# kamerkaya/SUPerman

Measured on AMD Instinct MI355X. Metric: Gray-code subset-steps/sec (dense n=40, d=0.5) at 1/2/4/8 MI355X; rel-err vs CPU, higher is better.
Workload: dtype f64; 1 GPU; dense Ryser/Gray-code exact permanent (-p4/-p6 path), n=40 d=0.50 (double/40_0.50_0), 2^39 Gray steps per step; n=40, kernel_request=dense, preprocessing=0, jit=1, walk=segmented (pattern-specialised), parallelism=dp1: contiguous wave-chunk shards + one RCCL all-reduce

## Files before the change

### include/superman.h

```cpp
#ifndef SUPERMAN_H
#define SUPERMAN_H

#include <stddef.h>
#include <stdint.h>

#ifdef __cplusplus
extern "C" {
#endif

#define SUP_ABI_VERSION 15

#define SUP_OK            0
#define SUP_EINVAL      (-1)
#define SUP_ENODEV      (-2)
#define SUP_EHIP        (-3)
#define SUP_ERCCL       (-4)
#define SUP_ENOMEM      (-5)
#define SUP_EIO         (-6)
#define SUP_EUNSUPPORTED (-7)

#define SUP_MAX_N 64
#define SUP_MAX_READ_N 4096

typedef enum {
  SUP_INT32 = 0,
  SUP_FLOAT32 = 1,
  SUP_FLOAT64 = 2
} sup_dtype;

typedef enum {
  SUP_KERNEL_DENSE = 0,
  SUP_KERNEL_SPARYSER = 1,
  SUP_KERNEL_SKIPPER = 2,
  SUP_KERNEL_DENSE_PLAIN = 3,
  SUP_KERNEL_SEGMENTED = 4,
  SUP_KERNEL_DENSE_LDS = 5
} sup_kernel;

typedef enum {
  SUP_SCHED_SINGLE = 0,
  SUP_SCHED_STATIC = 1,
  SUP_SCHED_CHUNKS = 2,
  SUP_SCHED_MANUAL = 3
} sup_sched;

typedef struct {
  int gpu_num;
  int device_id;
  int threads;
  int cpu_worker;
  int grid_dim;
  int block_dim;
  int walk_log2;
  int chunk_log2;
  int use_rccl;
  int verbose;
  int jit;
  const char* checkpoint;
  int timing;
} sup_opts;

typedef struct {
  double   kernel_ms;
  double   wall_ms;
  uint64_t gray_steps;
  uint64_t visited_steps;
  int      devices_used;
  int      lane_bits;
  int      walk_bits;
  int      grid;
  int      chunks_done_cpu;
  double   partials[16];
  int      walk_kind;
  int      leaves;
  double   est_ops_per_step;
  double   jit_ms;
  int      items_resumed;
  int16_t  seg_cached_bits;
  int16_t  seg_pair_bits;
} sup_stats;

void sup_opts_init(sup_opts* o);

int         sup_abi_version(void);
const char* sup_last_error(void);
int         sup_device_count(int* count);
int         sup_rccl_devices(int ndev, int* phys);
uint64_t    sup_device_checks(void);
int         sup_device_warmup(int device_id, int gpu_num, int n);
int         sup_kernel_time(int device_id, double* total_ms, uint64_t* launches);

int sup_perman(const void* mat, sup_dtype t, int n, sup_kernel kernel, sup_sched sched,
               const sup_opts* o, double* out, sup_stats* st);

int sup_partial(const void* mat, sup_dtype t, int n, sup_kernel kernel,
                uint64_t start, uint64_t end, const sup_opts* o, double* out, sup_stats* st);

int sup_perman_shard(const void* mat, sup_dtype t, int n, sup_kernel kernel, int shard, int nshards,
                     const sup_opts* o, double* out_partial, sup_stats* st);

int sup_plan_info(const void* mat, sup_dtype t, int n, sup_kernel kernel, const sup_opts* o, int* walk_kind,
                  int* colmap, int* lane_bits, int* walk_bits, int* cached_bits, int* pair_bits,
                  double* est_ops_per_step);

int sup_plan_key(const void* mat, sup_dtype t, int n, sup_kernel kernel, const sup_opts* o, uint64_t* key);

int sup_prepare(const void* mat, sup_dtype t, int n, sup_kernel kernel, const sup_opts* o, int* walk_kind,
                double* compile_ms);
int sup_perman_cpu(const void* mat, sup_dtype t, int n, sup_kernel kernel, int threads,
                   double* out, sup_stats* st);

int sup_perman_exact(const void* mat, sup_dtype t, int n, const sup_opts* o, int on_cpu, char* out,
                     size_t out_len, sup_stats* st);

int sup_perman_exact_range(const void* mat, sup_dtype t, int n, uint64_t c0, uint64_t c1, const sup_opts* o,
                           int on_cpu, int form, int group, uint64_t* primes, uint64_t* residues, int cap,
                           int* nprimes, int* colmap, sup_stats* st);

int sup_perman_quad(const void* mat, sup_dtype t, int n, const sup_opts* o, int on_cpu, double* out_hi,
                    double* out_lo, sup_stats* st);

int sup_perman_quad_range(const void* mat, sup_dtype t, int n, uint64_t c0, uint64_t c1, const sup_opts* o,
                          int on_cpu, int form, double* out_hi, double* out_lo, int* colmap, sup_stats* st);

int sup_perman_complex(const double* mat, int n, const sup_opts* o, int on_cpu,
                       double* out_re, double* out_im, sup_stats* st);
int sup_perman_complex_range(const double* mat, int n, uint64_t c0, uint64_t c1,
                             const sup_opts* o, int on_cpu,
                             double* out_re, double* out_im, sup_stats* st);

int sup_perman_complex_batch(const double* mats, int n, uint64_t count, const sup_opts* o,
                             int on_cpu, double* out, sup_stats* st);
int sup_perman_complex_submatrices(const double* U, int R, int C, const int32_t* rows,
                                   const int32_t* cols, int n, uint64_t count, const sup_opts* o,
                                   int on_cpu, double* out, sup_stats* st);

int sup_perman_complex_fock(const double* U, int R, int C, const int32_t* rows,
                            const int32_t* cols, int n, uint64_t count, const sup_opts* o,
                            int on_cpu, double* out, sup_stats* st);
int sup_perman_complex_fock_plan(const int32_t* rows, const int32_t* cols, int n,
                                 uint64_t count, uint64_t* terms, int* side);

int sup_perman_complex_minors(const double* U, int R, int C, const int32_t* rows, const int32_t* cols,
                              int n, uint64_t count, const sup_opts* o, int on_cpu, double* out, sup_stats* st);
int sup_perman_complex_minors_range(const double* mat, int n, uint64_t c0, uint64_t c1, const sup_opts* o,
                                    int on_cpu, double* out, sup_stats* st);
int sup_boson_sample(const double* U, int M, const int32_t* inputs, int n, uint64_t nsamples, uint64_t seed,
                     const sup_opts* o, int on_cpu, int32_t* out , sup_stats* st);

int sup_nw_start(const void* mat, sup_dtype t, int n, double* x0, double* p0);


int sup_gpu_perman64_xshared_coalescing_mshared(const void* mat, sup_dtype t, int nov,
    int grid_dim, int block_dim, double* out);
int sup_gpu_perman64_xshared_coalescing_mshared_multigpu(const void* mat, sup_dtype t, int nov,
    int gpu_num, int grid_dim, int block_dim, double* out);
int sup_gpu_perman64_xshared_coalescing_mshared_multigpucpu_chunks(const void* mat, sup_dtype t,
    int nov, int gpu_num, int cpu, int threads, int grid_dim, int block_dim, double* out);
int sup_gpu_perman64_xshared_coalescing_mshared_sparse(const void* mat, const int* cptrs,
    const int* rows, const void* cvals, sup_dtype t, int nov, int grid_dim, int block_dim,
    double* out);
int sup_gpu_perman64_xshared_coalescing_mshared_multigpu_sparse(const void* mat, const int* cptrs,
    const int* rows, const void* cvals, sup_dtype t, int nov, int gpu_num, int grid_dim,
    int block_dim, double* out);
int sup_gpu_perman64_xshared_coalescing_mshared_multigpucpu_chunks_sparse(const void* mat,
    const int* cptrs, const int* rows, const void* cvals, sup_dtype t, int nov, int gpu_num,
    int cpu, int threads, int grid_dim, int block_dim, double* out);
int sup_gpu_perman64_xshared_coalescing_mshared_multigpu_manual_distribution(const void* mat, sup_dtype t,
    int nov, int gpu_num, int grid_dim, int block_dim, double* out);
int sup_gpu_perman64_xshared_coalescing_mshared_multigpu_sparse_manual_distribution(const void* mat,
    const int* cptrs, const int* rows, const void* cvals, sup_dtype t, int nov, int gpu_num, int grid_dim,
    int block_dim, double* out);
int sup_gpu_perman64_xshared_coalescing_mshared_skipper(const void* mat, const int* rptrs,
    const int* cols, const int* cptrs, const int* rows, const void* cvals, sup_dtype t, int nov,
    int grid_dim, int block_dim, double* out);
int sup_gpu_perman64_xshared_coalescing_mshared_multigpucpu_chunks_skipper(const void* mat,
    const int* rptrs, const int* cols, const int* cptrs, const int* rows, const void* cvals,
    sup_dtype t, int nov, int gpu_num, int cpu, int threads, int grid_dim, int block_dim,
    double* out);


int sup_read_matrix(const char* path, int binary, void** mat, sup_dtype* t, int* n, int* nnz_header);
void sup_free(void* p);

int sup_count_nnz(const void* mat, sup_dtype t, int n, int* nnz);
int sup_compress(const void* mat, sup_dtype t, int n, int* cptrs, int* rows, void* cvals,
                 int* rptrs, int* cols, void* rvals);
int sup_sort_order(void* mat, sup_dtype t, int n, int* colperm);
int sup_skip_order(void* mat, sup_dtype t, int n, int* rowperm, int* colperm);

int sup_read_mtx(const char* path, int binary, void** mat, sup_dtype* t, int* n, int* nnz_lines);
int sup_read_mtx_complex(const char* path, double** mat, int* n, int* nnz_lines);

typedef struct {
  int compress;
  double scale_threshold;
  int min_n;
  int max_deg;
  int preprocessing;
} sup_reduce_opts;
void sup_reduce_opts_init(sup_reduce_opts* r);

typedef int (*sup_leaf_fn)(const double* a, int n, void* user, double* out_perm);

int sup_decompose(const void* mat, sup_dtype t, int n, const sup_reduce_opts* r, sup_leaf_fn fn, void* user,
                  double* out, int* n_leaves);

int sup_perman_reduced(const void* mat, sup_dtype t, int n, sup_kernel kernel, sup_sched sched, const sup_opts* o,
                       int on_cpu, const sup_reduce_opts* r, double* out, sup_stats* st);

int sup_perman_reduced_exact(const void* mat, sup_dtype t, int n, const sup_opts* o, int on_cpu,
                             const sup_reduce_opts* r, char* out, size_t out_len, sup_stats* st);

int sup_perman_reduced_quad(const void* mat, sup_dtype t, int n, const sup_opts* o, int on_cpu,
                            const sup_reduce_opts* r, double* out_hi, double* out_lo, sup_stats* st);



typedef struct {
  double   mean;
  double   std_error;
  double   zero_fraction;
  uint64_t samples;
  double   kernel_ms;
  double   wall_ms;
  int      devices;
  int      reserved_;
  int64_t  cpu_blocks;
} sup_approx_result;

int sup_approx(const void* mat, sup_dtype t, int n, int method, uint64_t samples, int scale_intervals,
               int scale_times, uint64_t seed, const sup_opts* o, int on_cpu, sup_approx_result* res);

int sup_grid_graph(int m, int n, int** mat, int* nov);

#ifdef __cplusplus
}
#endif
#endif
```

### superman_amd/__init__.py

```python
from __future__ import annotations

import ctypes as C
import os

import numpy as np

from . import _lib
from ._lib import (KERNEL_DENSE, KERNEL_SKIPPER, KERNEL_SPARYSER, LEAF_FN, SCHED_CHUNKS, SCHED_MANUAL, SCHED_SINGLE,
                   SCHED_STATIC, SupApproxResult, SupError, SupOpts, SupReduceOpts, SupStats)

__all__ = [
    "perman", "perman_cpu", "perman_exact", "perman_exact_range", "perman_quad", "perman_quad_range", "perman_complex", "perman_complex_range", "perman_complex_batch", "perman_complex_submatrices", "perman_complex_fock", "perman_complex_fock_plan", "perman_complex_minors", "perman_complex_minors_submatrices", "perman_complex_minors_range", "boson_sample", "read_mtx_complex", "partial", "perman_shard", "plan_info", "plan_key", "prepare", "read_matrix", "read_mtx", "sort_order",
    "skip_order", "compress", "decompose", "perman_reduced", "approx", "grid_graph", "ALGOS_APPROX",
    "nw_start", "device_count", "rccl_devices", "layout", "ShardCall", "SupError", "ALGOS_DENSE", "ALGOS_SPARSE",
    "gpu_perman64_xshared_coalescing_mshared",
    "gpu_perman64_xshared_coalescing_mshared_multigpu",
    "gpu_perman64_xshared_coalescing_mshared_multigpucpu_chunks",
    "gpu_perman64_xshared_coalescing_mshared_sparse",
    "gpu_perman64_xshared_coalescing_mshared_multigpu_sparse",
    "gpu_perman64_xshared_coalescing_mshared_multigpucpu_chunks_sparse",
    "gpu_perman64_xshared_coalescing_mshared_skipper",
    "gpu_perman64_xshared_coalescing_mshared_multigpucpu_chunks_skipper",
]

_DT = {np.dtype(np.int32): _lib.SUP_INT32, np.dtype(np.float32): _lib.SUP_FLOAT32,
       np.dtype(np.float64): _lib.SUP_FLOAT64}
_NP = {_lib.SUP_INT32: np.int32, _lib.SUP_FLOAT32: np.float32, _lib.SUP_FLOAT64: np.float64}
_TYPE_NAME = {_lib.SUP_INT32: "int", _lib.SUP_FLOAT32: "float", _lib.SUP_FLOAT64: "double"}

ALGOS_DENSE = {
    0: ("gpu_perman64_xglobal", KERNEL_DENSE, SCHED_SINGLE),
    1: ("gpu_perman64_xlocal", KERNEL_DENSE, SCHED_SINGLE),
    2: ("gpu_perman64_xshared", KERNEL_DENSE, SCHED_SINGLE),
    3: ("gpu_perman64_xshared_coalescing", KERNEL_DENSE, SCHED_SINGLE),
    4: ("gpu_perman64_xshared_coalescing_mshared", KERNEL_DENSE, SCHED_SINGLE),
    5: ("gpu_perman64_xshared_coalescing_mshared_multigpu", KERNEL_DENSE, SCHED_STATIC),
    6: ("gpu_perman64_xshared_coalescing_mshared_multigpucpu_chunks", KERNEL_DENSE, SCHED_CHUNKS),
    66: ("gpu_perman64_xshared_coalescing_mshared_multigpu_manual_distribution", KERNEL_DENSE, SCHED_MANUAL),
}
ALGOS_SPARSE = {
    1: ("gpu_perman64_xlocal_sparse", KERNEL_SPARYSER, SCHED_SINGLE),
    2: ("gpu_perman64_xshared_sparse", KERNEL_SPARYSER, SCHED_SINGLE),
    3: ("gpu_perman64_xshared_coalescing_sparse", KERNEL_SPARYSER, SCHED_SINGLE),
    4: ("gpu_perman64_xshared_coalescing_mshared_sparse", KERNEL_SPARYSER, SCHED_SINGLE),
    5: ("gpu_perman64_xshared_coalescing_mshared_multigpu_sparse", KERNEL_SPARYSER, SCHED_STATIC),
    6: ("gpu_perman64_xshared_coalescing_mshared_multigpucpu_chunks_sparse", KERNEL_SPARYSER, SCHED_CHUNKS),
    7: ("gpu_perman64_xshared_coalescing_mshared_skipper", KERNEL_SKIPPER, SCHED_SINGLE),
    8: ("gpu_perman64_xshared_coalescing_mshared_multigpucpu_chunks_skipper", KERNEL_SKIPPER, SCHED_CHUNKS),
    66: ("gpu_perman64_xshared_coalescing_mshared_multigpu_sparse_manual_distribution", KERNEL_SPARYSER,
         SCHED_MANUAL),
}
_KERNELS = {"dense": KERNEL_DENSE, "sparse": KERNEL_SPARYSER, "spa": KERNEL_SPARYSER,
            "skipper": KERNEL_SKIPPER, "skip": KERNEL_SKIPPER, "dense_plain": _lib.KERNEL_DENSE_PLAIN,
            "seg": _lib.KERNEL_SEGMENTED, "segmented": _lib.KERNEL_SEGMENTED,
            "dense_lds": _lib.KERNEL_DENSE_LDS}
WALK_NAMES = {0: "dense", 1: "sparse", 2: "skip", 3: "seg", 4: "lds"}


def _mat(a, max_n: int = 64) -> tuple[np.ndarray, int, int]:
    a = np.asarray(a)
    if a.dtype not in _DT:
        a = a.astype(np.float64)
    a = np.ascontiguousarray(a)
    if a.ndim != 2 or a.shape[0] != a.shape[1]:
        raise ValueError(f"expected a square matrix, got shape {a.shape}")
    n = a.shape[0]
    if not 1 <= n <= max_n:
        raise ValueError(f"n = {n} outside [1, {max_n}]" + (" (64-bit Gray index)" if max_n == 64 else ""))
    return a, _DT[a.dtype], n


def _opts(gpu_num=1, device_id=0, threads=16, cpu=False, walk_log2=0, chunk_log2=0, use_rccl=False,
          verbose=False, jit=0, checkpoint=None) -> SupOpts:
    lib = _lib.load()
    o = SupOpts()
    lib.sup_opts_init(C.byref(o))
    o.gpu_num, o.device_id, o.threads = int(gpu_num), int(device_id), int(threads)
    o.cpu_worker, o.walk_log2, o.chunk_log2 = int(bool(cpu)), int(walk_log2), int(chunk_log2)
    o.use_rccl, o.verbose = int(use_rccl), int(bool(verbose))
    o.jit = int(jit)
    o.checkpoint = os.fsencode(checkpoint) if checkpoint else None
    return o


def device_count() -> int:
    lib = _lib.load()
    c = C.c_int(0)
    rc = lib.sup_device_count(C.byref(c))
    return c.value if rc == 0 else 0


def rccl_devices(ndev: int) -> list:
    lib = _lib.load()
    out = (C.c_int * max(1, ndev))()
    _lib.check(lib.sup_rccl_devices(ndev, out), "rccl_devices")
    return list(out[:ndev])


def layout(n: int) -> tuple[int, int, int]:
    nb = n - 1
    L = min(6, nb)
    rest = nb - L
    m = min(rest, 10)
    if rest - m < 13:
        m = max(min(rest, 6), rest - 13)
    m = min(max(m, rest - 20), 31)
    return L, m, rest - m


def perman(mat, algo: int = 4, sparse: bool = False, gpu_num: int = 1, cpu: bool = False,
           threads: int = 16, device_id: int = 0, use_rccl: bool = False, walk_log2: int = 0,
           chunk_log2: int = 0, return_stats: bool = False, jit: int = 0, kernel: str | None = None,
           checkpoint: str | None = None):
    table = ALGOS_SPARSE if sparse else ALGOS_DENSE
    if algo not in table:
        raise SupError(-7, "perman", f"unknown algorithm id {algo}")
    _, kern, sched = table[algo]
    if kernel is not None:
        kern = _KERNELS[kernel]
    if algo == 66 and gpu_num == 1:
        gpu_num = 4
    if sched == SCHED_SINGLE:
        gpu_num = 1
    a, dt, n = _mat(mat)
    lib = _lib.load()
    o = _opts(gpu_num, device_id, threads, cpu, walk_log2, chunk_log2, use_rccl, jit=jit, checkpoint=checkpoint)
    out, st = C.c_double(0.0), SupStats()
    _lib.check(lib.sup_perman(a.ctypes.data, dt, n, kern, sched, C.byref(o), C.byref(out), C.byref(st)),
               table[algo][0])
    return (out.value, st.as_dict()) if return_stats else out.value


def perman_cpu(mat, kernel: str = "dense", threads: int = 16, return_stats: bool = False):
    a, dt, n = _mat(mat)
    lib = _lib.load()
    out, st = C.c_double(0.0), SupStats()
    _lib.check(lib.sup_perman_cpu(a.ctypes.data, dt, n, _KERNELS[kernel], int(threads), C.byref(out),
                                  C.byref(st)), "perman_cpu")
    return (out.value, st.as_dict()) if return_stats else out.value


def perman_exact(mat, gpu_num: int = 1, device_id: int = 0, cpu: bool = False, threads: int = 16,
                 return_stats: bool = False, cpu_worker: bool = False, chunk_log2: int = 0):
    a, dt, n = _mat(mat)
    lib = _lib.load()
    o = _opts(gpu_num=gpu_num, device_id=device_id, threads=threads, cpu=cpu_worker, chunk_log2=chunk_log2)
    buf = C.create_string_buffer(1024)
    st = SupStats()
    _lib.check(lib.sup_perman_exact(a.ctypes.data, dt, n, C.byref(o), int(bool(cpu)), buf, len(buf), C.byref(st)),
               "perman_exact")
    v = int(buf.value.decode())
    return (v, st.as_dict()) if return_stats else v


def perman_quad(mat, gpu_num: int = 1, device_id: int = 0, cpu: bool = False, threads: int = 16,
                return_stats: bool = False):
    a, dt, n = _mat(mat)
    lib = _lib.load()
    o = _opts(gpu_num=gpu_num, device_id=device_id, threads=threads)
    hi, lo, st = C.c_double(0.0), C.c_double(0.0), SupStats()
    _lib.check(lib.sup_perman_quad(a.ctypes.data, dt, n, C.byref(o), int(bool(cpu)), C.byref(hi), C.byref(lo),
                                   C.byref(st)), "perman_quad")
    return ((hi.value, lo.value), st.as_dict()) if return_stats else (hi.value, lo.value)


# ... 182 lines not shown
    out, st = np.zeros(2 * n), SupStats()
    src = b if b.size else np.zeros(2)
    _lib.check(lib.sup_perman_complex_minors_range(src.ctypes.data, n, int(c0), int(c1), C.byref(o), int(bool(cpu)),
                                                   out.ctypes.data, C.byref(st)), "perman_complex_minors_range")
    v = _batch_result(out, n)
    return (v, st.as_dict()) if return_stats else v


def boson_sample(U, inputs, nsamples: int, seed: int = 0, gpu_num: int = 1, device_id: int = 0, cpu: bool = False,
                 threads: int = 16, walk_log2: int = 0, return_stats: bool = False):
    u = np.ascontiguousarray(np.asarray(U, dtype=np.complex128))
    if u.ndim != 2 or u.shape[0] != u.shape[1] or u.shape[0] < 1:
        raise ValueError(f"expected a square matrix U, got shape {u.shape}")
    ins = np.asarray(inputs)
    if ins.ndim != 1 or ins.size < 1:
        raise ValueError(f"inputs must be a non-empty 1-d list of modes, got shape {ins.shape}")
    if not np.issubdtype(ins.dtype, np.integer):
        raise ValueError(f"inputs must be integers, got dtype {ins.dtype}")
    if ins.min() < -2**31 or ins.max() >= 2**31:
        raise ValueError("inputs holds a mode outside the 32-bit range")
    i32 = np.ascontiguousarray(ins, dtype=np.int32)
    nsamples, n = int(nsamples), int(i32.size)
    if nsamples < 0:
        raise ValueError("nsamples must be >= 0")
    lib = _lib.load()
    o = _opts(gpu_num=gpu_num, device_id=device_id, threads=threads, walk_log2=walk_log2)
    out, st = np.zeros((max(nsamples, 1), n), np.int32), SupStats()
    _lib.check(lib.sup_boson_sample(u.ctypes.data, u.shape[0], i32.ctypes.data, n, nsamples,
                                    int(seed) & 0xFFFFFFFFFFFFFFFF, C.byref(o), int(bool(cpu)), out.ctypes.data,
                                    C.byref(st)), "boson_sample")
    v = out[:nsamples].copy()
    if not return_stats:
        return v
    d = st.as_dict()
    d["minors_ms"], d["pmf_ms"] = float(st.partials[0]), float(st.partials[1])
    return v, d


def _fock_lists(rows, cols):
    r, c = np.asarray(rows), np.asarray(cols)
    single = r.ndim == 1
    if single:
        r, c = r[None, :], c[None, :] if c.ndim == 1 else c
    if r.ndim != 2 or r.shape != c.shape:
        raise ValueError(f"rows and cols must both have shape [n] or [count, n], got {np.shape(rows)} and "
                         f"{np.shape(cols)}")
    for name, ix in (("rows", r), ("cols", c)):
        if ix.size and not np.issubdtype(ix.dtype, np.integer):
            raise ValueError(f"{name} must be an integer array, got dtype {ix.dtype}")
        if ix.size and (ix.min() < -2**31 or ix.max() >= 2**31):
            raise ValueError(f"{name} holds an index outside the 32-bit range")
    count, n = r.shape
    if not 1 <= n <= 64:
        raise ValueError(f"n = {n} outside [1, 64] (64-bit Gray index)")
    r32 = np.ascontiguousarray(r, dtype=np.int32) if count else np.zeros(1, np.int32)
    c32 = np.ascontiguousarray(c, dtype=np.int32) if count else np.zeros(1, np.int32)
    return r32, c32, count, n, single


def perman_complex_fock(U, rows, cols, gpu_num: int = 1, device_id: int = 0, cpu: bool = False, threads: int = 16,
                        return_stats: bool = False):
    u = np.ascontiguousarray(np.asarray(U, dtype=np.complex128))
    if u.ndim != 2 or u.shape[0] < 1 or u.shape[1] < 1:
        raise ValueError(f"expected a non-empty 2-d matrix U, got shape {u.shape}")
    r32, c32, count, n, single = _fock_lists(rows, cols)
    lib = _lib.load()
    o = _opts(gpu_num=gpu_num, device_id=device_id, threads=threads)
    out, st = np.zeros(2 * max(count, 1)), SupStats()
    _lib.check(lib.sup_perman_complex_fock(u.ctypes.data, u.shape[0], u.shape[1], r32.ctypes.data, c32.ctypes.data,
                                           n, count, C.byref(o), int(bool(cpu)), out.ctypes.data, C.byref(st)),
               "perman_complex_fock")
    v = _batch_result(out, count)
    v = complex(v[0]) if single else v
    return (v, st.as_dict()) if return_stats else v


def perman_complex_fock_plan(rows, cols):
    r32, c32, count, n, single = _fock_lists(rows, cols)
    lib = _lib.load()
    terms, side = np.zeros(max(count, 1), np.uint64), np.zeros(max(count, 1), np.int32)
    _lib.check(lib.sup_perman_complex_fock_plan(r32.ctypes.data, c32.ctypes.data, n, count, terms.ctypes.data,
                                                side.ctypes.data), "perman_complex_fock_plan")
    if single:
        return int(terms[0]), int(side[0])
    return terms[:count].copy(), side[:count].copy()


def partial(mat, start: int, end: int, kernel: str = "dense", gpu_num: int = 1, device_id: int = 0,
            walk_log2: int = 0, return_stats: bool = False):
    a, dt, n = _mat(mat)
    lib = _lib.load()
    o = _opts(gpu_num=gpu_num, device_id=device_id, walk_log2=walk_log2)
    out, st = C.c_double(0.0), SupStats()
    _lib.check(lib.sup_partial(a.ctypes.data, dt, n, _KERNELS[kernel], int(start), int(end), C.byref(o),
                               C.byref(out), C.byref(st)), "partial")
    return (out.value, st.as_dict()) if return_stats else out.value


def perman_shard(mat, shard: int, nshards: int, kernel: str = "dense", device_id: int = 0,
                 return_stats: bool = False, jit: int = 0, walk_log2: int = 0):
    a, dt, n = _mat(mat)
    lib = _lib.load()
    o = _opts(device_id=device_id, jit=jit, walk_log2=walk_log2)
    out, st = C.c_double(0.0), SupStats()
    _lib.check(lib.sup_perman_shard(a.ctypes.data, dt, n, _KERNELS[kernel], int(shard), int(nshards), C.byref(o),
                                    C.byref(out), C.byref(st)), "perman_shard")
    return (out.value, st.as_dict()) if return_stats else out.value


class ShardCall:

    def __init__(self, mat, shard: int, nshards: int, kernel: str = "dense", device_id: int = 0, jit: int = 0,
                 walk_log2: int = 0, timing: bool = True):
        self._a, dt, n = _mat(mat)
        self._lib = _lib.load()
        self._o = _opts(device_id=device_id, jit=jit, walk_log2=walk_log2)
        self._o.timing = int(bool(timing))
        self._out, self._st = C.c_double(0.0), SupStats()
        self._fn = self._lib.sup_perman_shard
        self._args = (self._a.ctypes.data, dt, n, _KERNELS[kernel], int(shard), int(nshards), C.byref(self._o),
                      C.byref(self._out), C.byref(self._st))

    def __call__(self):
        rc = self._fn(*self._args)
        if rc:
            _lib.check(rc, "perman_shard")
        return self._out.value, self._st.kernel_ms

    def stats(self) -> dict:
        return self._st.as_dict()


def kernel_time(device_id: int = 0):
    lib = _lib.load()
    ms, cnt = C.c_double(0.0), C.c_uint64(0)
    _lib.check(lib.sup_kernel_time(int(device_id), C.byref(ms), C.byref(cnt)), "kernel_time")
    return ms.value, cnt.value


def plan_info(mat, kernel: str = "dense", jit: int = 0, gpu_num: int = 1, device_id: int = 0,
              walk_log2: int = 0) -> dict:
    a, dt, n = _mat(mat)
    lib = _lib.load()
    kind, L, m, cc, pb = C.c_int(), C.c_int(), C.c_int(), C.c_int(), C.c_int()
    ops = C.c_double(0.0)
    cm = np.zeros(max(n - 1, 1), np.int32)
    o = _opts(gpu_num=gpu_num, device_id=device_id, jit=jit, walk_log2=walk_log2)
    _lib.check(lib.sup_plan_info(a.ctypes.data, dt, n, _KERNELS[kernel], C.byref(o), C.byref(kind), cm.ctypes.data,
                                 C.byref(L), C.byref(m), C.byref(cc), C.byref(pb), C.byref(ops)), "plan_info")
    return {"kind": WALK_NAMES[kind.value], "colmap": cm[: n - 1].copy(), "L": L.value, "m": m.value,
            "cached": cc.value, "pair_bits": pb.value, "est_ops_per_step": ops.value}


def plan_key(mat, kernel: str = "dense", jit: int = 0, gpu_num: int = 1, device_id: int = 0,
             walk_log2: int = 0) -> int:
    a, dt, n = _mat(mat)
    lib = _lib.load()
    key = C.c_uint64(0)
    o = _opts(gpu_num=gpu_num, device_id=device_id, jit=jit, walk_log2=walk_log2)
    _lib.check(lib.sup_plan_key(a.ctypes.data, dt, n, _KERNELS[kernel], C.byref(o), C.byref(key)), "plan_key")
    return key.value


def prepare(mat, kernel: str = "dense", jit: int = 0, gpu_num: int = 1, device_id: int = 0,
            walk_log2: int = 0) -> dict:
    a, dt, n = _mat(mat)
    lib = _lib.load()
    kind, ms = C.c_int(), C.c_double(0.0)
    o = _opts(gpu_num=gpu_num, device_id=device_id, jit=jit, walk_log2=walk_log2)
    _lib.check(lib.sup_prepare(a.ctypes.data, dt, n, _KERNELS[kernel], C.byref(o), C.byref(kind), C.byref(ms)),
               "prepare")
    return {"kind": WALK_NAMES[kind.value], "compile_ms": ms.value}


def nw_start(mat) -> tuple[np.ndarray, float]:
    a, dt, n = _mat(mat)
    lib = _lib.load()
    x0 = np.zeros(n, np.float64)
    p0 = C.c_double(0.0)
    _lib.check(lib.sup_nw_start(a.ctypes.data, dt, n, x0.ctypes.data_as(C.POINTER(C.c_double)), C.byref(p0)),
               "nw_start")
    return x0, p0.value


def read_matrix(path: str, binary: bool = False) -> tuple[np.ndarray, str, int]:
    lib = _lib.load()
    p, t, n, nnz = C.c_void_p(), C.c_int(), C.c_int(), C.c_int()
    _lib.check(lib.sup_read_matrix(path.encode(), int(bool(binary)), C.byref(p), C.byref(t), C.byref(n),
                                   C.byref(nnz)), "read_matrix")
    try:
        dtype = _NP[t.value]
        buf = (C.c_char * (n.value * n.value * np.dtype(dtype).itemsize)).from_address(p.value)
        m = np.frombuffer(buf, dtype=dtype).reshape(n.value, n.value).copy()
    finally:
        lib.sup_free(p)
    return m, _TYPE_NAME[t.value], nnz.value


def sort_order(mat) -> tuple[np.ndarray, np.ndarray]:
    a, dt, n = _mat(mat)
    a = a.copy()
    cp = np.zeros(n, np.int32)
    _lib.check(_lib.load().sup_sort_order(a.ctypes.data, dt, n, cp.ctypes.data), "sort_order")
    return a, cp


def skip_order(mat) -> tuple[np.ndarray, np.ndarray, np.ndarray]:
    a, dt, n = _mat(mat)
    a = a.copy()
    rp, cp = np.zeros(n, np.int32), np.zeros(n, np.int32)
    _lib.check(_lib.load().sup_skip_order(a.ctypes.data, dt, n, rp.ctypes.data, cp.ctypes.data), "skip_order")
    return a, rp, cp


def compress(mat) -> dict:
    a, dt, n = _mat(mat)
    lib = _lib.load()
    nnz = C.c_int(0)
    _lib.check(lib.sup_count_nnz(a.ctypes.data, dt, n, C.byref(nnz)), "count_nnz")
    k = max(nnz.value, 1)
    out = {"cptrs": np.zeros(n + 1, np.int32), "rows": np.zeros(k, np.int32), "cvals": np.zeros(k, a.dtype),
           "rptrs": np.zeros(n + 1, np.int32), "cols": np.zeros(k, np.int32), "rvals": np.zeros(k, a.dtype)}
    _lib.check(lib.sup_compress(a.ctypes.data, dt, n, *(out[f].ctypes.data for f in
                                                        ("cptrs", "rows", "cvals", "rptrs", "cols", "rvals"))),
               "compress")
    for f in ("rows", "cvals", "cols", "rvals"):
        out[f] = out[f][: nnz.value]
    return out


def gpu_perman64_xshared_coalescing_mshared(mat, grid_dim=2048, block_dim=256):
    return perman(mat, 4)


def gpu_perman64_xshared_coalescing_mshared_multigpu(mat, gpu_num, grid_dim=2048, block_dim=256):
    return perman(mat, 5, gpu_num=gpu_num)


def gpu_perman64_xshared_coalescing_mshared_multigpucpu_chunks(mat, gpu_num, cpu=False, threads=16,
                                                               grid_dim=2048, block_dim=256):
    return perman(mat, 6, gpu_num=gpu_num, cpu=cpu, threads=threads)


def gpu_perman64_xshared_coalescing_mshared_sparse(mat, grid_dim=2048, block_dim=256):
    return perman(mat, 4, sparse=True)


def gpu_perman64_xshared_coalescing_mshared_multigpu_sparse(mat, gpu_num, grid_dim=2048, block_dim=256):
    return perman(mat, 5, sparse=True, gpu_num=gpu_num)


def gpu_perman64_xshared_coalescing_mshared_multigpucpu_chunks_sparse(mat, gpu_num, cpu=False, threads=16,
                                                                      grid_dim=2048, block_dim=256):
    return perman(mat, 6, sparse=True, gpu_num=gpu_num, cpu=cpu, threads=threads)


def gpu_perman64_xshared_coalescing_mshared_skipper(mat, grid_dim=2048, block_dim=256):
    return perman(mat, 7, sparse=True)


def gpu_perman64_xshared_coalescing_mshared_multigpucpu_chunks_skipper(mat, gpu_num, cpu=False, threads=16,
                                                                       grid_dim=2048, block_dim=256):
    return perman(mat, 8, sparse=True, gpu_num=gpu_num, cpu=cpu, threads=threads)


def _reduce_opts(compress=True, scale=None, min_n=30, max_deg=5, preprocessing=0) -> SupReduceOpts:
    lib = _lib.load()
    r = SupReduceOpts()
    lib.sup_reduce_opts_init(C.byref(r))
    r.compress = int(bool(compress))
    r.scale_threshold = float(scale) if scale else 0.0
    r.min_n, r.max_deg, r.preprocessing = int(min_n), int(max_deg), int(preprocessing)
    return r


def decompose(mat, leaf, compress: bool = True, scale=None, min_n: int = 30, max_deg: int = 5):
    a, dt, n = _mat(mat, 4096)
    lib = _lib.load()
    seen, err = [], []

    def cb(ptr, k, _user, out):
        try:
            m = np.ctypeslib.as_array(ptr, shape=(k * k,)).reshape(k, k).copy()
            seen.append(m)
            out[0] = float(leaf(m))
            return 0
        except Exception as e:
            err.append(e)
            return -1

    fn = LEAF_FN(cb)
    r = _reduce_opts(compress, scale, min_n, max_deg)
    out, nl = C.c_double(0.0), C.c_int(0)
    rc = lib.sup_decompose(a.ctypes.data, dt, n, C.byref(r), fn, None, C.byref(out), C.byref(nl))
    if err:
        raise err[0]
    _lib.check(rc, "decompose")
    return out.value, seen


def perman_reduced(mat, algo: int = 4, sparse: bool = False, compress: bool = True, scale=None,
                   preprocessing: int = 0, gpu_num: int = 1, cpu: bool = False, threads: int = 16,
                   device_id: int = 0, min_n: int = 30, max_deg: int = 5, return_stats: bool = False):
    table = ALGOS_SPARSE if sparse else ALGOS_DENSE
    if algo not in table:
        raise SupError(-7, "perman_reduced", f"unknown algorithm id {algo}")
# ... 98 lines not shown
```

### superman_amd/_lib.py

```python
from __future__ import annotations

import ctypes as C
import os
import subprocess
import threading

PKG_DIR = os.path.dirname(os.path.abspath(__file__))
CSRC = os.path.join(PKG_DIR, "csrc")
LIB_PATH = os.path.join(PKG_DIR, "lib", "libsuperman_hip.so")
PERMAN_BIN = os.path.join(PKG_DIR, "bin", "perman")

SUP_OK = 0
ERRORS = {
    -1: "SUP_EINVAL",
    -2: "SUP_ENODEV",
    -3: "SUP_EHIP",
    -4: "SUP_ERCCL",
    -5: "SUP_ENOMEM",
    -6: "SUP_EIO",
    -7: "SUP_EUNSUPPORTED",
}
SUP_INT32, SUP_FLOAT32, SUP_FLOAT64 = 0, 1, 2
KERNEL_DENSE, KERNEL_SPARYSER, KERNEL_SKIPPER, KERNEL_DENSE_PLAIN, KERNEL_SEGMENTED, KERNEL_DENSE_LDS = 0, 1, 2, 3, 4, 5
SCHED_SINGLE, SCHED_STATIC, SCHED_CHUNKS, SCHED_MANUAL = 0, 1, 2, 3

EXPORTS = [
    "sup_opts_init", "sup_abi_version", "sup_last_error", "sup_device_count", "sup_rccl_devices", "sup_device_checks", "sup_device_warmup", "sup_kernel_time",
    "sup_perman", "sup_partial", "sup_perman_cpu", "sup_nw_start", "sup_perman_shard", "sup_plan_info",
    "sup_prepare", "sup_plan_key", "sup_perman_exact", "sup_perman_exact_range", "sup_perman_reduced_exact",
    "sup_perman_quad", "sup_perman_quad_range",
    "sup_perman_reduced_quad", "sup_perman_complex", "sup_perman_complex_range", "sup_read_mtx_complex",
    "sup_perman_complex_batch", "sup_perman_complex_submatrices",
    "sup_perman_complex_fock", "sup_perman_complex_fock_plan",
    "sup_perman_complex_minors", "sup_perman_complex_minors_range", "sup_boson_sample",
    "sup_gpu_perman64_xshared_coalescing_mshared",
    "sup_gpu_perman64_xshared_coalescing_mshared_multigpu",
    "sup_gpu_perman64_xshared_coalescing_mshared_multigpucpu_chunks",
    "sup_gpu_perman64_xshared_coalescing_mshared_multigpu_manual_distribution",
    "sup_gpu_perman64_xshared_coalescing_mshared_multigpu_sparse_manual_distribution",
    "sup_gpu_perman64_xshared_coalescing_mshared_sparse",
    "sup_gpu_perman64_xshared_coalescing_mshared_multigpu_sparse",
    "sup_gpu_perman64_xshared_coalescing_mshared_multigpucpu_chunks_sparse",
    "sup_gpu_perman64_xshared_coalescing_mshared_skipper",
    "sup_gpu_perman64_xshared_coalescing_mshared_multigpucpu_chunks_skipper",
    "sup_read_matrix", "sup_free", "sup_count_nnz", "sup_compress",
    "sup_sort_order", "sup_skip_order", "sup_read_mtx",
    "sup_reduce_opts_init", "sup_decompose", "sup_perman_reduced", "sup_approx", "sup_grid_graph",
]


class SupOpts(C.Structure):
    _fields_ = [
        ("gpu_num", C.c_int), ("device_id", C.c_int), ("threads", C.c_int),
        ("cpu_worker", C.c_int), ("grid_dim", C.c_int), ("block_dim", C.c_int),
        ("walk_log2", C.c_int), ("chunk_log2", C.c_int), ("use_rccl", C.c_int),
        ("verbose", C.c_int), ("jit", C.c_int), ("checkpoint", C.c_char_p), ("timing", C.c_int),
    ]


class SupReduceOpts(C.Structure):
    _fields_ = [
        ("compress", C.c_int), ("scale_threshold", C.c_double), ("min_n", C.c_int),
        ("max_deg", C.c_int), ("preprocessing", C.c_int),
    ]


class SupApproxResult(C.Structure):
    _fields_ = [
        ("mean", C.c_double), ("std_error", C.c_double), ("zero_fraction", C.c_double),
        ("samples", C.c_uint64), ("kernel_ms", C.c_double), ("wall_ms", C.c_double),
        ("devices", C.c_int), ("reserved_", C.c_int), ("cpu_blocks", C.c_int64),
    ]

    def as_dict(self) -> dict:
        return {f: getattr(self, f) for f, _ in self._fields_ if f != "reserved_"}


LEAF_FN = C.CFUNCTYPE(C.c_int, C.POINTER(C.c_double), C.c_int, C.c_void_p, C.POINTER(C.c_double))


class SupStats(C.Structure):
    _fields_ = [
        ("kernel_ms", C.c_double), ("wall_ms", C.c_double),
        ("gray_steps", C.c_uint64), ("visited_steps", C.c_uint64),
        ("devices_used", C.c_int), ("lane_bits", C.c_int), ("walk_bits", C.c_int),
        ("grid", C.c_int), ("chunks_done_cpu", C.c_int), ("partials", C.c_double * 16),
        ("walk_kind", C.c_int), ("leaves", C.c_int), ("est_ops_per_step", C.c_double),
        ("jit_ms", C.c_double), ("items_resumed", C.c_int), ("seg_cached_bits", C.c_int16),
        ("seg_pair_bits", C.c_int16),
    ]

    def as_dict(self) -> dict:
        d = {f: getattr(self, f) for f, _ in self._fields_ if f != "partials"}
        d["partials"] = list(self.partials[: max(1, self.devices_used)])
        return d


class SupError(RuntimeError):
    def __init__(self, code: int, what: str, msg: str):
        super().__init__(f"{what}: {ERRORS.get(code, code)}: {msg}")
        self.code = code


_lock = threading.Lock()
_lib = None


def build(quiet: bool = True) -> None:
    jobs = str(min(16, os.cpu_count() or 4))
    r = subprocess.run(["make", "-C", CSRC, "-j", jobs], capture_output=True, text=True)
    if r.returncode != 0:
        raise RuntimeError("building libsuperman_hip.so failed:\n" + r.stdout[-4000:] + r.stderr[-4000:])
    if not quiet:
        print(r.stdout)


def load() -> C.CDLL:
    global _lib
    with _lock:
        if _lib is not None:
            return _lib
        if not os.path.exists(LIB_PATH) or not os.path.exists(PERMAN_BIN):
            build()
        lib = C.CDLL(LIB_PATH)
        _declare(lib)
        if lib.sup_abi_version() != 15:
            raise RuntimeError("libsuperman_hip.so ABI version mismatch")
        _lib = lib
        return lib


def _declare(lib: C.CDLL) -> None:
    P, I, D = C.c_void_p, C.c_int, C.c_double
    lib.sup_opts_init.argtypes = [C.POINTER(SupOpts)]
    lib.sup_opts_init.restype = None
    lib.sup_abi_version.restype = I
    lib.sup_last_error.restype = C.c_char_p
    lib.sup_device_count.argtypes = [C.POINTER(I)]
    lib.sup_rccl_devices.argtypes = [I, C.POINTER(I)]
    lib.sup_device_checks.restype = C.c_uint64
    lib.sup_device_warmup.argtypes = [I, I, I]
    lib.sup_kernel_time.restype = I
    lib.sup_kernel_time.argtypes = [I, C.POINTER(C.c_double), C.POINTER(C.c_uint64)]
    lib.sup_perman.argtypes = [P, I, I, I, I, C.POINTER(SupOpts), C.POINTER(D), C.POINTER(SupStats)]
    lib.sup_partial.argtypes = [P, I, I, I, C.c_uint64, C.c_uint64, C.POINTER(SupOpts), C.POINTER(D),
                                C.POINTER(SupStats)]
    lib.sup_perman_cpu.argtypes = [P, I, I, I, I, C.POINTER(D), C.POINTER(SupStats)]
    lib.sup_perman_exact.argtypes = [P, I, I, C.POINTER(SupOpts), I, C.c_char_p, C.c_size_t, C.POINTER(SupStats)]
    lib.sup_perman_quad.argtypes = [P, I, I, C.POINTER(SupOpts), I, C.POINTER(D), C.POINTER(D), C.POINTER(SupStats)]
    lib.sup_perman_exact_range.argtypes = [P, I, I, C.c_uint64, C.c_uint64, C.POINTER(SupOpts), I, I, I, P, P, I,
                                           C.POINTER(I), P, C.POINTER(SupStats)]
    lib.sup_perman_quad_range.argtypes = [P, I, I, C.c_uint64, C.c_uint64, C.POINTER(SupOpts), I, I, C.POINTER(D),
                                          C.POINTER(D), P, C.POINTER(SupStats)]
    lib.sup_perman_complex.argtypes = [P, I, C.POINTER(SupOpts), I, C.POINTER(D), C.POINTER(D), C.POINTER(SupStats)]
    lib.sup_perman_complex_range.argtypes = [P, I, C.c_uint64, C.c_uint64, C.POINTER(SupOpts), I, C.POINTER(D),
                                             C.POINTER(D), C.POINTER(SupStats)]
    lib.sup_perman_complex_batch.argtypes = [P, I, C.c_uint64, C.POINTER(SupOpts), I, P, C.POINTER(SupStats)]
    lib.sup_perman_complex_submatrices.argtypes = [P, I, I, P, P, I, C.c_uint64, C.POINTER(SupOpts), I, P,
                                                   C.POINTER(SupStats)]
    lib.sup_perman_complex_fock.argtypes = [P, I, I, P, P, I, C.c_uint64, C.POINTER(SupOpts), I, P,
                                            C.POINTER(SupStats)]
    lib.sup_perman_complex_fock_plan.argtypes = [P, P, I, C.c_uint64, P, P]
    lib.sup_perman_complex_minors.argtypes = [P, I, I, P, P, I, C.c_uint64, C.POINTER(SupOpts), I, P,
                                              C.POINTER(SupStats)]
    lib.sup_perman_complex_minors_range.argtypes = [P, I, C.c_uint64, C.c_uint64, C.POINTER(SupOpts), I, P,
                                                    C.POINTER(SupStats)]
    lib.sup_boson_sample.argtypes = [P, I, P, I, C.c_uint64, C.c_uint64, C.POINTER(SupOpts), I, P,
                                     C.POINTER(SupStats)]
    lib.sup_read_mtx_complex.argtypes = [C.c_char_p, C.POINTER(P), C.POINTER(I), C.POINTER(I)]
    lib.sup_perman_shard.argtypes = [P, I, I, I, I, I, C.POINTER(SupOpts), C.POINTER(D), C.POINTER(SupStats)]
    lib.sup_plan_info.argtypes = [P, I, I, I, C.POINTER(SupOpts), C.POINTER(I), P, C.POINTER(I), C.POINTER(I),
                                  C.POINTER(I), C.POINTER(I), C.POINTER(D)]
    lib.sup_prepare.argtypes = [P, I, I, I, C.POINTER(SupOpts), C.POINTER(I), C.POINTER(C.c_double)]
    lib.sup_plan_key.argtypes = [P, I, I, I, C.POINTER(SupOpts), C.POINTER(C.c_uint64)]
    lib.sup_nw_start.argtypes = [P, I, I, C.POINTER(D), C.POINTER(D)]
    lib.sup_read_matrix.argtypes = [C.c_char_p, I, C.POINTER(P), C.POINTER(I), C.POINTER(I), C.POINTER(I)]
    lib.sup_free.argtypes = [P]
    lib.sup_free.restype = None
    lib.sup_count_nnz.argtypes = [P, I, I, C.POINTER(I)]
    lib.sup_compress.argtypes = [P, I, I, P, P, P, P, P, P]
    lib.sup_sort_order.argtypes = [P, I, I, P]
    lib.sup_skip_order.argtypes = [P, I, I, P, P]
    lib.sup_approx.argtypes = [P, I, I, I, C.c_uint64, I, I, C.c_uint64, C.POINTER(SupOpts), I,
                               C.POINTER(SupApproxResult)]
    lib.sup_grid_graph.argtypes = [I, I, C.POINTER(C.POINTER(C.c_int)), C.POINTER(I)]
    lib.sup_read_mtx.argtypes = [C.c_char_p, I, C.POINTER(P), C.POINTER(I), C.POINTER(I), C.POINTER(I)]
    lib.sup_reduce_opts_init.argtypes = [C.POINTER(SupReduceOpts)]
    lib.sup_reduce_opts_init.restype = None
    lib.sup_decompose.argtypes = [P, I, I, C.POINTER(SupReduceOpts), LEAF_FN, P, C.POINTER(D), C.POINTER(I)]
    lib.sup_perman_reduced_exact.argtypes = [P, I, I, C.POINTER(SupOpts), I, C.POINTER(SupReduceOpts), C.c_char_p,
                                             C.c_size_t, C.POINTER(SupStats)]
    lib.sup_perman_reduced_quad.argtypes = [P, I, I, C.POINTER(SupOpts), I, C.POINTER(SupReduceOpts), C.POINTER(D),
                                            C.POINTER(D), C.POINTER(SupStats)]
    lib.sup_perman_reduced.argtypes = [P, I, I, I, I, C.POINTER(SupOpts), I, C.POINTER(SupReduceOpts),
                                       C.POINTER(D), C.POINTER(SupStats)]
    for name in EXPORTS:
        if name not in ("sup_opts_init", "sup_free", "sup_last_error", "sup_reduce_opts_init"):
            getattr(lib, name).restype = I


def check(rc: int, what: str) -> None:
    if rc != SUP_OK:
        msg = _lib.sup_last_error().decode(errors="replace") if _lib is not None else ""
        raise SupError(rc, what, msg)
```

### superman_amd/csrc/capi.cpp

```cpp
#include <algorithm>
#include <chrono>
#include <cstdlib>
#include <cstring>
#include <mutex>

#include "dd.hpp"
#include "engine.hpp"

using namespace sup;

namespace {

int check_common(const void* mat, int n, double* out) {
  if (!mat || !out) {
    set_error("null matrix or output pointer");
    return SUP_EINVAL;
  }
  if (n < 1 || n > SUP_MAX_N) {
    set_error("n = " + std::to_string(n) + " outside [1, 64] (64-bit Gray index)");
    return SUP_EINVAL;
  }
  return SUP_OK;
}

// ... 461 lines not shown
  auto t0 = std::chrono::steady_clock::now();
  if (!U || !rows || !cols || !out) {
    set_error("sup_perman_complex_fock: null matrix, index list or output pointer");
    return SUP_EINVAL;
  }
  sup_opts o;
  if (o_in) o = *o_in;
  else sup_opts_init(&o);
  CplxBatchIn in;
  in.U = U, in.R = R, in.C = C, in.rows = rows, in.cols = cols;
  FockInfo fi;
  if (int rc = cplx_perman_fock(in, n, count, o, on_cpu != 0, out, &fi)) return rc;
  if (st) {
    std::memset(st, 0, sizeof(*st));
    st->kernel_ms = fi.kernel_ms;
    st->wall_ms = std::chrono::duration<double, std::milli>(std::chrono::steady_clock::now() - t0).count();
    st->gray_steps = count << (n - 1);
    st->visited_steps = fi.terms;
    st->devices_used = fi.devices;
    st->grid = fi.grid;
    st->walk_kind = (int)kWalkDense;
    st->leaves = (int)std::min<uint64_t>(count, 0x7fffffffu);
    st->est_ops_per_step = 6.0 * n;
  }
  return SUP_OK;
}

int sup_perman_complex_fock_plan(const int32_t* rows, const int32_t* cols, int n, uint64_t count, uint64_t* terms,
                                 int* side) {
  return cplx_fock_plan(rows, cols, n, count, terms, side);
}

static void fill_minors_stats(sup_stats* st, const CplxInfo& ci, int n, uint64_t outputs, uint64_t steps,
                              double wall_ms) {
  fill_cplx_stats(st, ci, n, steps, wall_ms);
  if (!st) return;
  st->leaves = (int)std::min<uint64_t>(outputs, 0x7fffffffu);
  st->est_ops_per_step = n <= 32 ? std::max(16.0 * n - 24.0, 0.0) : 6.0 * (n - 1);
}

int sup_perman_complex_minors(const double* U, int R, int C, const int32_t* rows, const int32_t* cols, int n,
                              uint64_t count, const sup_opts* o_in, int on_cpu, double* out, sup_stats* st) {
  auto t0 = std::chrono::steady_clock::now();
  if (!U || !rows || (!cols && n != 1) || !out) {
    set_error("sup_perman_complex_minors: null matrix, index list or output pointer");
    return SUP_EINVAL;
  }
  sup_opts o;
  if (o_in) o = *o_in;
  else sup_opts_init(&o);
  CplxBatchIn in;
  in.U = U, in.R = R, in.C = C, in.rows = rows, in.cols = cols;
  CplxInfo ci;
  if (int rc = cplx_minors(in, n, count, o, on_cpu != 0, out, &ci)) return rc;
  const double wall = std::chrono::duration<double, std::milli>(std::chrono::steady_clock::now() - t0).count();
  const uint64_t per = n <= 1 ? 0 : n <= 32 ? 1ull << (n - 2) : (uint64_t)n << (n - 2);
  fill_minors_stats(st, ci, n, count * (uint64_t)n, count * per, wall);
  return SUP_OK;
}

int sup_perman_complex_minors_range(const double* mat, int n, uint64_t c0, uint64_t c1, const sup_opts* o_in,
                                    int on_cpu, double* out, sup_stats* st) {
  auto t0 = std::chrono::steady_clock::now();
  sup_opts o;
  if (o_in) o = *o_in;
  else sup_opts_init(&o);
  CplxInfo ci;
  if (int rc = cplx_minors_range(mat, n, c0, c1, o, on_cpu != 0, out, &ci)) return rc;
  const double wall = std::chrono::duration<double, std::milli>(std::chrono::steady_clock::now() - t0).count();
  fill_minors_stats(st, ci, n, 1, (c1 - c0) << (ci.lay.L + ci.lay.m), wall);
  return SUP_OK;
}

int sup_boson_sample(const double* U, int M, const int32_t* inputs, int n, uint64_t nsamples, uint64_t seed,
                     const sup_opts* o_in, int on_cpu, int32_t* out, sup_stats* st) {
  auto t0 = std::chrono::steady_clock::now();
  sup_opts o;
  if (o_in) o = *o_in;
  else sup_opts_init(&o);
  BosonInfo bi;
  if (int rc = boson_sample(U, M, inputs, n, nsamples, seed, o, on_cpu != 0, out, &bi)) return rc;
  if (st) {
    std::memset(st, 0, sizeof(*st));
    st->kernel_ms = bi.kernel_ms;
    st->wall_ms = std::chrono::duration<double, std::milli>(std::chrono::steady_clock::now() - t0).count();
    st->gray_steps = bi.steps;
    st->visited_steps = bi.steps;
    st->devices_used = bi.devices;
    st->walk_kind = (int)kWalkDense;
    st->leaves = (int)std::min<uint64_t>(nsamples, 0x7fffffffu);
    st->est_ops_per_step = std::max(16.0 * n - 24.0, 0.0);
    st->partials[0] = bi.minors_ms;
    st->partials[1] = bi.pmf_ms;
  }
  return SUP_OK;
}

int sup_perman_reduced_exact(const void* mat, sup_dtype t, int n, const sup_opts* o_in, int on_cpu,
                             const sup_reduce_opts* r_in, char* out, size_t out_len, sup_stats* st) {
  auto t0 = std::chrono::steady_clock::now();
  if (!mat || !out || out_len < 2 || n < 1 || n > SUP_MAX_READ_N) {
    set_error("sup_perman_reduced_exact: bad argument");
    return SUP_EINVAL;
  }
  const size_t nn = (size_t)n * n;
  std::vector<double> A(nn);
  for (size_t i = 0; i < nn; ++i)
    A[i] = t == SUP_INT32 ? (double)((const int32_t*)mat)[i]
           : t == SUP_FLOAT32 ? (double)((const float*)mat)[i] : ((const double*)mat)[i];
  sup_opts o;
  if (o_in) o = *o_in;
  else sup_opts_init(&o);
  sup_reduce_opts r;
  if (r_in) r = *r_in;
  else sup_reduce_opts_init(&r);
  std::string s;
  double kms = 0.0;
  int leaves = 0, rc;
  if ((rc = exact_perman_reduced(A.data(), n, o, on_cpu != 0, r, s, &kms, &leaves))) return rc;
  if (s.size() + 1 > out_len) {
    set_error("sup_perman_reduced_exact: output buffer too small");
    return SUP_EINVAL;
  }
  std::memcpy(out, s.c_str(), s.size() + 1);
  if (st) {
    std::memset(st, 0, sizeof(*st));
    st->kernel_ms = kms;
    st->wall_ms = std::chrono::duration<double, std::milli>(std::chrono::steady_clock::now() - t0).count();
    st->leaves = leaves;
    st->walk_kind = (int)kWalkDense;
  }
  return SUP_OK;
}

int sup_plan_info(const void* mat, sup_dtype t, int n, sup_kernel kernel, const sup_opts* o_in, int* walk_kind,
                  int* colmap, int* L, int* m, int* cached_bits, int* pair_bits, double* est_ops_per_step) {
  std::vector<double> A;
  int rc = to_double(mat, t, n, A);
  if (rc) return rc;
  sup_opts o;
  if (o_in) o = *o_in;
  else sup_opts_init(&o);
  Plan P;
  if ((rc = check_walk_opts(o))) return rc;
  if ((rc = plan_for(A.data(), n, kernel, layout_for(n, o), P, o.jit, o.gpu_num, o.device_id))) return rc;
  if (walk_kind) *walk_kind = P.lds ? 4 : (int)P.kind;
  if (cached_bits) *cached_bits = P.kind == kWalkSeg ? P.seg_cc : 0;
  if (pair_bits) *pair_bits = P.kind == kWalkSeg ? P.seg_b : 0;
  if (est_ops_per_step) *est_ops_per_step = walk_cost(P);
  if (colmap)
    for (int e = 0; e < n - 1; ++e) colmap[e] = P.colmap[e];
  if (L) *L = P.lay.L;
  if (m) *m = P.lay.m;
  return SUP_OK;
}

int sup_plan_key(const void* mat, sup_dtype t, int n, sup_kernel kernel, const sup_opts* o_in, uint64_t* key) {
  if (!key) {
    set_error("sup_plan_key: key pointer missing");
    return SUP_EINVAL;
  }
  std::vector<double> A;
  int rc = to_double(mat, t, n, A);
  if (rc) return rc;
  sup_opts o;
  if (o_in) o = *o_in;
  else sup_opts_init(&o);
  Plan P;
  if ((rc = check_walk_opts(o))) return rc;
  if ((rc = plan_for(A.data(), n, kernel, layout_for(n, o), P, o.jit, o.gpu_num, o.device_id))) return rc;
  *key = plan_fingerprint(P);
  return SUP_OK;
}

int sup_prepare(const void* mat, sup_dtype t, int n, sup_kernel kernel, const sup_opts* o_in, int* walk_kind,
                double* compile_ms) {
  std::vector<double> A;
  int rc = to_double(mat, t, n, A);
  if (rc) return rc;
  sup_opts o;
  if (o_in) o = *o_in;
  else sup_opts_init(&o);
  Plan P;
  if ((rc = check_walk_opts(o))) return rc;
  const double before = jit_compile_ms_thread();
  if ((rc = plan_for(A.data(), n, kernel, layout_for(n, o), P, o.jit, o.gpu_num, o.device_id))) return rc;
  if (walk_kind) *walk_kind = P.lds ? 4 : (int)P.kind;
  if (P.kind == kWalkSeg && (rc = jit_compile_only(P, nullptr))) return rc;
  if (compile_ms) *compile_ms = jit_compile_ms_thread() - before;
  return SUP_OK;
}

static double entry(const void* mat, sup_dtype t, size_t i) {
  return t == SUP_INT32 ? (double)((const int32_t*)mat)[i]
         : t == SUP_FLOAT32 ? (double)((const float*)mat)[i] : ((const double*)mat)[i];
}

static int check_compressed(const void* mat, sup_dtype t, int n, const int* cptrs, const int* rows,
                            const void* cvals, const int* rptrs, const int* cols) {
  if (!mat || n < 1 || n > SUP_MAX_N) {
    set_error("reference wrapper: null matrix or n outside [1, 64]");
    return SUP_EINVAL;
  }
  if (!cptrs || !rows || !cvals) {
    set_error("reference wrapper: CSC arrays (cptrs, rows, cvals) missing");
    return SUP_EINVAL;
  }
  auto bad = [](const std::string& m) {
    set_error("reference wrapper: " + m + " (build CSR/CSC with sup_compress: nonzero test != 0)");
    return SUP_EINVAL;
  };
  if (cptrs[0] != 0) return bad("cptrs[0] != 0");
  for (int c = 0; c < n; ++c) {
    if (cptrs[c + 1] < cptrs[c]) return bad("cptrs not ascending");
    int want = 0;
    for (int r = 0; r < n; ++r) want += entry(mat, t, (size_t)r * n + c) != 0.0;
    if (cptrs[c + 1] - cptrs[c] != want)
      return bad("column " + std::to_string(c) + " lists " + std::to_string(cptrs[c + 1] - cptrs[c]) +
                 " entries, the matrix has " + std::to_string(want) + " nonzeros");
    for (int k = cptrs[c]; k < cptrs[c + 1]; ++k) {
      const int r = rows[k];
      if (r < 0 || r >= n || (k > cptrs[c] && r <= rows[k - 1])) return bad("CSC rows out of range or order");
      const double v = entry(mat, t, (size_t)r * n + c);
      if (v == 0.0 || entry(cvals, t, (size_t)k) != v)
        return bad("CSC value at (" + std::to_string(r) + ", " + std::to_string(c) + ") differs from the matrix");
    }
  }
  if (rptrs || cols) {
    if (!rptrs || !cols) return bad("CSR arrays incomplete");
    if (rptrs[0] != 0) return bad("rptrs[0] != 0");
    for (int r = 0; r < n; ++r) {
      if (rptrs[r + 1] < rptrs[r]) return bad("rptrs not ascending");
      int want = 0;
      for (int c = 0; c < n; ++c) want += entry(mat, t, (size_t)r * n + c) != 0.0;
      if (rptrs[r + 1] - rptrs[r] != want) return bad("row " + std::to_string(r) + " nonzero count differs");
      for (int k = rptrs[r]; k < rptrs[r + 1]; ++k) {
        const int c = cols[k];
        if (c < 0 || c >= n || (k > rptrs[r] && c <= cols[k - 1]) || entry(mat, t, (size_t)r * n + c) == 0.0)
          return bad("CSR columns out of range, order or pattern");
      }
    }
  }
  return SUP_OK;
}

static int run_ref(const void* mat, sup_dtype t, int nov, sup_kernel k, sup_sched s, int gpu_num, int cpu,
                   int threads, double* out) {
  sup_opts o;
  sup_opts_init(&o);
  o.gpu_num = gpu_num < 1 ? 1 : gpu_num;
  o.cpu_worker = cpu;
  o.threads = threads;
  return sup_perman(mat, t, nov, k, s, &o, out, nullptr);
}

int sup_gpu_perman64_xshared_coalescing_mshared(const void* mat, sup_dtype t, int nov, int, int, double* out) {
  return run_ref(mat, t, nov, SUP_KERNEL_DENSE, SUP_SCHED_SINGLE, 1, 0, 16, out);
}
int sup_gpu_perman64_xshared_coalescing_mshared_multigpu(const void* mat, sup_dtype t, int nov, int gpu_num, int,
                                                         int, double* out) {
  return run_ref(mat, t, nov, SUP_KERNEL_DENSE, SUP_SCHED_STATIC, gpu_num, 0, 16, out);
}
int sup_gpu_perman64_xshared_coalescing_mshared_multigpucpu_chunks(const void* mat, sup_dtype t, int nov,
                                                                   int gpu_num, int cpu, int threads, int, int,
                                                                   double* out) {
  return run_ref(mat, t, nov, SUP_KERNEL_DENSE, SUP_SCHED_CHUNKS, gpu_num, cpu, threads, out);
}
int sup_gpu_perman64_xshared_coalescing_mshared_multigpu_manual_distribution(const void* mat, sup_dtype t, int nov,
                                                                             int gpu_num, int, int, double* out) {
  return run_ref(mat, t, nov, SUP_KERNEL_DENSE, SUP_SCHED_MANUAL, gpu_num, 0, 16, out);
}
int sup_gpu_perman64_xshared_coalescing_mshared_sparse(const void* mat, const int* cptrs, const int* rows,
                                                       const void* cvals, sup_dtype t, int nov, int, int,
                                                       double* out) {
  int rc = check_compressed(mat, t, nov, cptrs, rows, cvals, nullptr, nullptr);
  return rc ? rc : run_ref(mat, t, nov, SUP_KERNEL_SPARYSER, SUP_SCHED_SINGLE, 1, 0, 16, out);
}
int sup_gpu_perman64_xshared_coalescing_mshared_multigpu_sparse(const void* mat, const int* cptrs, const int* rows,
                                                                const void* cvals, sup_dtype t, int nov, int gpu_num,
                                                                int, int, double* out) {
  int rc = check_compressed(mat, t, nov, cptrs, rows, cvals, nullptr, nullptr);
  return rc ? rc : run_ref(mat, t, nov, SUP_KERNEL_SPARYSER, SUP_SCHED_STATIC, gpu_num, 0, 16, out);
}
int sup_gpu_perman64_xshared_coalescing_mshared_multigpucpu_chunks_sparse(const void* mat, const int* cptrs,
                                                                          const int* rows, const void* cvals,
                                                                          sup_dtype t, int nov, int gpu_num, int cpu,
                                                                          int threads, int, int, double* out) {
  int rc = check_compressed(mat, t, nov, cptrs, rows, cvals, nullptr, nullptr);
  return rc ? rc : run_ref(mat, t, nov, SUP_KERNEL_SPARYSER, SUP_SCHED_CHUNKS, gpu_num, cpu, threads, out);
}
int sup_gpu_perman64_xshared_coalescing_mshared_multigpu_sparse_manual_distribution(const void* mat, const int* cptrs,
                                                                                    const int* rows, const void* cvals,
                                                                                    sup_dtype t, int nov, int gpu_num,
                                                                                    int, int, double* out) {
  int rc = check_compressed(mat, t, nov, cptrs, rows, cvals, nullptr, nullptr);
  return rc ? rc : run_ref(mat, t, nov, SUP_KERNEL_SPARYSER, SUP_SCHED_MANUAL, gpu_num, 0, 16, out);
}
int sup_gpu_perman64_xshared_coalescing_mshared_skipper(const void* mat, const int* rptrs, const int* cols,
                                                        const int* cptrs, const int* rows, const void* cvals,
                                                        sup_dtype t, int nov, int, int, double* out) {
  int rc = check_compressed(mat, t, nov, cptrs, rows, cvals, rptrs, cols);
  return rc ? rc : run_ref(mat, t, nov, SUP_KERNEL_SKIPPER, SUP_SCHED_SINGLE, 1, 0, 16, out);
}
int sup_gpu_perman64_xshared_coalescing_mshared_multigpucpu_chunks_skipper(const void* mat, const int* rptrs,
                                                                           const int* cols, const int* cptrs,
                                                                           const int* rows, const void* cvals,
// ... 260 lines not shown
```

### superman_amd/csrc/engine.hpp

```cpp
#pragma once
#include <stdint.h>
#include <cstdio>
#include <memory>
#include <mutex>
#include <functional>
#include <string>
#include <vector>

#include "../../include/superman.h"
#include "kernels.hpp"

namespace sup {

void set_error(const std::string& msg);
const char* last_error();
bool env_on(const char* name, bool dflt);

int to_double(const void* mat, sup_dtype t, int n, std::vector<double>& out);

void nw_start(const double* A, int n, double* x0, double* p0);

constexpr int kMaxCachedBits = 4;

struct Layout {
  int L;
  int m;
  int h;
  bool fixed = false;
  int cc_cap = kMaxCachedBits;
  uint64_t chunks() const { return 1ull << h; }
};
Layout default_layout(int n);
Layout layout_with_walk(int n, int walk_log2);

struct ProdTree {
  std::vector<int> item_row;
  std::vector<uint32_t> item_sig;
  int tail_lo = 0, tail_hi = 0;
  std::vector<int> a, b;
  std::vector<uint32_t> sig;
  std::vector<uint8_t> item_live, node_live;
  int items() const { return (int)item_row.size(); }
  int K() const { return (int)a.size(); }
  int root() const { return K() ? items() + K() - 1 : (items() ? 0 : -1); }
  uint32_t root_sig() const { return K() ? sig.back() : (items() ? item_sig[0] : 0u); }
};

struct Plan {
  int n = 0;
  int NP = 0;
  WalkKind kind = kWalkDense;
  Layout lay{};
  std::vector<int> rowperm;
  std::vector<int> colmap;
  std::vector<double> cols;
  std::vector<double> x0;
  std::vector<int> nblk;
  std::vector<uint64_t> rowmask;
  uint64_t umask = 0;
  uint64_t chunk_ends = 0;
  std::vector<int> seg_start;
  std::vector<std::vector<int>> touched;
  std::vector<int> sub_start;
  int seg_b = 0;
  std::vector<int> dyn_rows;
  ProdTree outer_tree;
  ProdTree inner_tree;
  bool lds = false;
  bool integral = false;
  int seg_cc = 0;
  double seg_ops = 0.0;
  double seg_skip = 0.0;
  int seg_regs = 0;
  int seg_budget = 0;
  std::vector<int> jofs;
  std::vector<double> jtab;
  size_t seg_cbase = 0;
  bool start_tab_on = false;
  std::vector<double> start_tab;
  int seg_kp = 4;
  std::string jit_src;
  uint64_t jit_key = 0;
  uint64_t uid = 0;
  std::vector<int> seg_order;
  bool seg_loop_scratch = false;
};

struct SegChoice {
  std::vector<int> order;
  int b = 0;
  int budget = 0;
  int cc_cap = kMaxCachedBits;
};

int make_plan(const double* A, int n, WalkKind kind, bool identity_map, const Layout& lay, Plan& P,
              const SegChoice* choice = nullptr);

std::vector<int> greedy_walk_order(const double* A, int n, int count);
bool skip_walk_order(const double* A, int n, const Layout& lay, std::vector<int>& out,
                     const std::vector<int>* baseline, double factor);
int improve_sparse_plan(const double* A, int n, const Layout& lay, Plan& P);
int plan_threads();

std::vector<int> seg_walk_order(const double* A, int n, int m, int count, int* b_out, int cc_cap = kMaxCachedBits);
double seg_skip_estimate(const double* A, int n, const std::vector<int>& order, int m, int samples);
double seg_skip_fraction_plan(const Plan& P, int samples);
std::vector<int> seg_row_order(const double* A, int n, const std::vector<int>& walk);
int build_seg(Plan& P, int fixed_budget = 0);
bool seg_choice_load(uint64_t key, int* m, SegChoice* c);
bool seg_choice_exists(uint64_t key);
double seg_cold_model(int n);
double seg_cold_predict(int n);
void seg_cost_store(int n, double seconds);
double seg_cost_ratio_load();
void seg_choice_store(uint64_t key, int m, const SegChoice& c);
int auto_decision_load(uint64_t key);
int auto_decision_store(uint64_t key, int seg);
uint64_t jit_toolchain_hash();
int seg_static_bits(int m);
double seg_cx(const Plan& P, int r, uint32_t S);
double seg_cy(const Plan& P, int r, uint32_t S);
double seg_walk_cost(const Plan& P);
int jit_occupancy(int dev, const Plan& P, int* blocks_per_cu, double* compile_ms);
int jit_launch(int dev, const Plan& P, const WalkParams& p, int grid, hipStream_t s);
int jit_compile_only(const Plan& P, double* compile_ms);
struct CodeScan {
  int vgprs = -1, vgpr_spills = -1, scratch_bytes = -1;
  int insts = 0, scratch_insts = 0, loops = 0;
  int loop_scratch = -1, loop_f64 = 0, loop_insts = 0;
  int loop_readlane = 0;
};
int scan_code_object(const std::vector<char>& code, const char* kernel, CodeScan* out);
int jit_code_scan(const Plan& P, CodeScan* out);
double jit_compile_ms_thread();

double walk_cost(const Plan& P);
double walk_seconds(const Plan& P, double steps);

int plan_for(const double* A, int n, sup_kernel kernel, const Layout& lay, Plan& P, int jit = -1, int ndev = 1,
             int dev = 0);
int plan_for_shared(const double* A, int n, sup_kernel kernel, const Layout& lay, std::shared_ptr<const Plan>& P,
                    int jit = -1, int ndev = 1, int dev = 0, bool keep = true);

struct RangeResult {
  double partial = 0.0;
  double kernel_ms = 0.0;
  uint64_t visited = 0;
  int grid = 0;
  double compile_ms = 0.0;
};

int run_item_queue(uint64_t nitems, int takers, const std::function<int(int, uint64_t)>& take);
int run_range(int dev, const Plan& P, uint64_t c0, uint64_t c1, bool want_visited, RangeResult& r,
              double* slot = nullptr);
struct LaunchGeom {
  unsigned group, tail_group;
  uint64_t tail_begin, grid;
  unsigned tail_ticket;
};
LaunchGeom walk_geometry(uint64_t count, uint64_t resident_blocks, uint64_t waves_per_block, bool seg,
                         int force_group = 0, int force_tail = -1, uint64_t group_cap = 64);
constexpr int kMaxBatchLeaves = 32;
constexpr int kMaxBatchLeafChunkBits = 26;
static_assert((uint64_t)kMaxBatchLeaves << kMaxBatchLeafChunkBits <= (1ull << 32),
              "leaf batches must fit 32-bit chunk indices");
bool batchable(const Plan& a, const Plan& b);
int run_range_batch(int dev, const std::vector<const Plan*>& plans, std::vector<double>& partial, double* kernel_ms);

double pairwise_host(const std::vector<double>& v);

int device_count(int* n);
constexpr int kCtxLanes = 8;
void set_ctx_lane(int lane);
int ctx_lane();
void set_defer_timing(bool on);
int kernel_time(int dev, double* total_ms, uint64_t* launches);
int phys_device(int dev);
hipError_t select_device(int dev);
int check_device(int dev, const char* what);
uint64_t device_checks_passed();
#ifndef SUP_HIP
#define SUP_HIP(call)                                                                  \
  do {                                                                                 \
    hipError_t e_ = (call);                                                            \
    if (e_ != hipSuccess) {                                                            \
      set_error(std::string(#call) + ": " + hipGetErrorString(e_));                    \
      return SUP_EHIP;                                                                 \
    }                                                                                  \
  } while (0)
#endif

#define SUP_ON_DEVICE(dev, what)                 \
  do {                                           \
    const int rc_ = check_device((dev), (what)); \
    if (rc_) return rc_;                         \
  } while (0)
int warm_devices(int first, int count, int n);
int rccl_physical_devices(const std::vector<int>& devs, std::vector<int>& phys);

struct SchedResult {
  double total = 0.0;
  double kernel_ms = 0.0;
  uint64_t visited = 0;
  int devices = 0;
  int grid = 0;
  int cpu_items = 0;
  double compile_ms = 0.0;
  int items_resumed = 0;
  std::vector<double> dev_partials;
};
int schedule(const Plan& P, sup_sched sched, const sup_opts& o, uint64_t c0, uint64_t c1,
             SchedResult& out);
struct Checkpoint {
  FILE* f = nullptr;
  std::mutex mu;
  ~Checkpoint() {
    if (f) std::fclose(f);
  }
};
int ckpt_open(const char* path, const char* head, uint64_t nitems, std::vector<double>& ipart,
              std::vector<char>& done, uint64_t& vis, int& resumed, Checkpoint& ck);
int ckpt_record(Checkpoint& ck, uint64_t it, double part, uint64_t visited);

uint64_t plan_fingerprint(const Plan& P);

double cpu_walk_range(const Plan& P, uint64_t c0, uint64_t c1, int threads);

int run_range_exact(int dev, const Plan& P, int group, uint64_t c0, uint64_t c1, const std::vector<double>& primes,
                    std::vector<uint64_t>& res, double* kernel_ms);
void cpu_exact_range(const Plan& P, uint64_t c0, uint64_t c1, const std::vector<double>& primes, int threads,
                     std::vector<uint64_t>& res);
struct RangeInfo {
  double kernel_ms = 0.0, est_ops = 0.0;
  int devices = 0;
  int walk_kind = 0;
  int group = 0;
  Layout lay{};
  std::vector<int> colmap;
};
int exact_perman(const double* A, int n, const sup_opts& o, bool on_cpu, std::string& out, double* kernel_ms,
                 int* devices_used, int* cpu_items = nullptr, RangeInfo* info = nullptr);
int check_range_request(int n, const sup_opts& o, int form, const char* who);
int exact_perman_range(const double* A, int n, uint64_t c0, uint64_t c1, const sup_opts& o, bool on_cpu, int form,
                       int group, int cap, std::vector<uint64_t>& primes, std::vector<uint64_t>& res,
                       RangeInfo* info);
int exact_perman_reduced(const double* A, int n, const sup_opts& o, bool on_cpu, const sup_reduce_opts& r,
                         std::string& out, double* kernel_ms, int* leaves);

int run_range_dd(int dev, const Plan& P, const std::vector<double>& x0dd, uint64_t c0, uint64_t c1,
                 double* parts, double* kernel_ms);
void cpu_dd_range(const Plan& P, const std::vector<double>& x0dd, uint64_t c0, uint64_t c1, int threads,
                  double* parts);
struct dd;
int decompose_batched(const double* A, int n, const sup_reduce_opts& r, int workers,
                      const std::function<int(int, const double*, int, double*)>& leaf, double* out, int* n_leaves,
                      bool memo = true);
typedef std::function<int(int, const std::vector<const double*>&, int, const std::vector<double*>&,
                          std::function<int()>&)>
    LeafBatchStagedFn;
int decompose_batched_staged(const double* A, int n, const sup_reduce_opts& r, int workers, int batch_max,
                             const LeafBatchStagedFn& staged, double* out, int* n_leaves);
// ... 73 lines not shown
```

### superman_amd/csrc/jit.cpp

```cpp
#include <dlfcn.h>
#include <hip/hiprtc.h>
#include <sched.h>
#include <spawn.h>
#include <sys/stat.h>
#include <sys/wait.h>
#include <unistd.h>

#include <cerrno>

#include <algorithm>
#include <cstring>
#include <fstream>
#include <iterator>
#include <atomic>
#include <chrono>
#include <cmath>
#include <cstdio>
#include <cstdlib>
#include <map>
#include <queue>
#include <memory>
#include <condition_variable>
#include <mutex>
#include <sstream>
// ... 561 lines not shown
          }
        size_t bi = 0;
        for (size_t i = 1; i < starts.size(); ++i)
          if (effs[i] < effs[bi] - 1e-12) bi = i;
        beff = effs[bi], bb = std::get<1>(starts[bi]), bo = std::get<2>(starts[bi]);
        if (std::getenv("SUP_JIT_VERBOSE")) std::fprintf(stderr, "  polished eff=%.4f\n", beff);
      }
      if (b_out) *b_out = bb;
      return bo;
    }
  }
  if (b_out) *b_out = cands[gi];
  return extend(bests[gi], count);
}

double seg_skip_fraction_plan(const Plan& P, int samples) {
  const int n = P.n, L = P.lay.L, m = P.lay.m, nb = n - 1;
  const int tail_lo = P.seg_start.empty() ? n : P.seg_start.back();
  if (tail_lo >= n) return 0.0;
  for (const double v : P.cols)
    if (v != std::floor(v)) return 0.0;
  const int h = nb - L - m;
  int skipped = 0;
  std::vector<double> base(n - tail_lo);
  for (int s = 0; s < samples; ++s) {
    const uint64_t a = h > 0 ? ((uint64_t)s * 0x9E3779B97F4A7C15ull) >> (64 - std::min(h, 63)) : 0;
    const uint64_t g = a ^ (a >> 1);
    for (int r = tail_lo; r < n; ++r) {
      double v = P.x0[r];
      for (int k = 0; k < h; ++k)
        if ((g >> k) & 1u) v += P.cols[(size_t)(2 * (L + m + k)) * P.NP + r];
      base[r - tail_lo] = v;
    }
    bool all = true;
    for (unsigned lane = 0; lane < (1u << L) && all; ++lane) {
      bool zero = false;
      for (int r = tail_lo; r < n && !zero; ++r) {
        double v = base[r - tail_lo];
        for (int e = 0; e < L; ++e)
          if ((lane >> e) & 1u) v += P.cols[(size_t)(2 * e) * P.NP + r];
        zero = v == 0.0;
      }
      all = zero;
    }
    skipped += all;
  }
  return (double)skipped / samples;
}

double seg_skip_estimate(const double* A, int n, const std::vector<int>& order, int m, int samples) {
  const int nb = n - 1, L = std::min(6, nb - m);
  if ((int)order.size() < m + L) return 0.0;
  std::vector<char> walk(n, 0), used(n, 0);
  for (int k = 0; k < m; ++k) walk[order[k]] = used[order[k]] = 1;
  for (int e = 0; e < L; ++e) used[order[m + e]] = 1;
  std::vector<int> high;
  for (int c = 0; c < nb; ++c)
    if (!used[c]) high.push_back(c);
  std::vector<int> tail;
  for (int r = 0; r < n; ++r) {
    bool t = true;
    for (int c = 0; c < nb && t; ++c) t = !(walk[c] && A[(size_t)r * n + c] != 0.0);
    if (t) tail.push_back(r);
  }
  if (tail.empty()) return 0.0;
  std::vector<double> x0(n);
  double p0;
  nw_start(A, n, x0.data(), &p0);
  const int h = (int)high.size();
  struct Row {
    double x0;
    std::vector<std::pair<int, double>> hi;
    std::vector<std::pair<double, uint64_t>> lane;
  };
  const uint64_t all_lanes = L >= 6 ? ~0ull : (1ull << (1u << L)) - 1ull;
  std::vector<Row> rows(tail.size());
  for (size_t i = 0; i < tail.size(); ++i) {
    const double* a = A + (size_t)tail[i] * n;
    rows[i].x0 = x0[tail[i]];
    for (int k = 0; k < h; ++k)
      if (a[high[k]] != 0.0) rows[i].hi.push_back({k, a[high[k]]});
    for (unsigned l = 0; l < (1u << L); ++l) {
      double v = 0.0;
      for (int e = 0; e < L; ++e)
        if ((l >> e) & 1u) v += a[order[m + e]];
      auto it = std::find_if(rows[i].lane.begin(), rows[i].lane.end(), [&](const auto& q) { return q.first == -v; });
      if (it == rows[i].lane.end()) rows[i].lane.push_back({-v, 1ull << l});
      else it->second |= 1ull << l;
    }
  }
  int skipped = 0;
  for (int s = 0; s < samples; ++s) {
    const uint64_t a = h ? ((uint64_t)s * 0x9E3779B97F4A7C15ull) >> (64 - std::min(h, 63)) : 0;
    const uint64_t g = a ^ (a >> 1);
    uint64_t zero = 0;
    for (size_t i = 0; i < rows.size() && zero != all_lanes; ++i) {
      double v = rows[i].x0;
      for (const auto& q : rows[i].hi)
        if ((g >> q.first) & 1u) v += q.second;
      for (const auto& q : rows[i].lane)
        if (v == q.first) zero |= q.second;
    }
    skipped += zero == all_lanes;
  }
  return (double)skipped / samples;
}

std::vector<int> seg_row_order(const double* A, int n, const std::vector<int>& walk) {
  std::vector<int> order;
  std::vector<char> placed(n, 0), in0(n, 0);
  for (int i = 0; i < n; ++i) in0[i] = !walk.empty() && A[(size_t)i * n + walk[0]] != 0.0;
  for (size_t k = 1; k < walk.size(); ++k)
    for (int i = 0; i < n; ++i)
      if (in0[i] && !placed[i] && A[(size_t)i * n + walk[k]] != 0.0) placed[i] = 1, order.push_back(i);
  for (int i = 0; i < n; ++i)
    if (in0[i] && !placed[i]) placed[i] = 1, order.push_back(i);
  for (size_t k = 1; k < walk.size(); ++k)
    for (int i = 0; i < n; ++i)
      if (!placed[i] && A[(size_t)i * n + walk[k]] != 0.0) placed[i] = 1, order.push_back(i);
  for (int i = 0; i < n; ++i)
    if (!placed[i]) order.push_back(i);
  return order;
}


double seg_cx(const Plan& P, int r, uint32_t S) {
  const uint32_t low = S & (0u - S), rest = S ^ low;
  const int k = __builtin_ctz(low) + 1;
  const double a = P.cols[(size_t)(2 * (P.lay.L + k)) * P.NP + r];
  return rest ? seg_cx(P, r, rest) + a : a;
}
double seg_cy(const Plan& P, int r, uint32_t S) {
  const double a0 = P.cols[(size_t)(2 * P.lay.L) * P.NP + r];
  return S ? a0 + seg_cx(P, r, S) : a0;
}

namespace {

std::string tree(int lo, int hi, const char* v = "x") {
  if (hi - lo == 1) return std::string(v) + "[" + std::to_string(lo) + "]";
  const int mid = lo + (hi - lo + 1) / 2;
  return "(" + tree(lo, mid, v) + " * " + tree(mid, hi, v) + ")";
}

std::vector<uint32_t> submasks(uint32_t m) {
  std::vector<uint32_t> v;
  for (uint32_t s = 0; s <= m; ++s)
    if ((s & ~m) == 0) v.push_back(s);
  return v;
}

struct Stmt {
  std::string text;
};

struct Gen {
  const Plan& P;
  int len0;
  uint32_t ccm;
  std::vector<uint32_t> rsig;
  std::ostringstream o;
  std::map<std::tuple<int, uint32_t, int>, int> cdir;
  std::vector<double> ctab;
  size_t cbase = 0;
  std::vector<int> kofs;
  std::vector<std::vector<int>> cpos;
  std::vector<char> own_stream;
  std::vector<std::vector<Stmt>> cls_stmts;
  std::vector<std::vector<double>> cls_consts;
  std::vector<std::pair<int, int>> item_of;

  explicit Gen(const Plan& p) : P(p), len0(p.seg_start[1]), ccm((1u << p.seg_cc) - 1u), rsig(p.n, 0u) {
    for (int k = 1; k < p.lay.m; ++k)
      for (int r : p.touched[k]) rsig[r] |= 1u << step_class(k, p.seg_b);
    item_of.assign(p.n, {-1, -1});
    for (int ti = 0; ti < 2; ++ti) {
      const ProdTree& t = ti ? p.inner_tree : p.outer_tree;
      for (int j = 0; j < t.items(); ++j)
        if (t.item_row[j] >= 0) item_of[t.item_row[j]] = {ti, j};
    }
  }
  const ProdTree& tr(int ti) const { return ti ? P.inner_tree : P.outer_tree; }
  uint32_t rs(int r) const { return rsig[r] & ccm; }
  bool live(int r, int v) const {
    const auto it = item_of[r];
    return it.first >= 0 && (tr(it.first).item_live[it.second] >> v) & 1u;
  }
  double cval(int r, uint32_t S, int v) const { return v ? seg_cy(P, r, S) : seg_cx(P, r, S); }
  std::string cname(int r, uint32_t S, int v) const {
    if (v == 0) return S ? "x" + std::to_string(r) + "_" + std::to_string(S) : "x[" + std::to_string(r) + "]";
    return S ? "y" + std::to_string(r) + "_" + std::to_string(S) : "y[" + std::to_string(r) + "]";
  }
  int dir(int r, uint32_t S, int v) {
    auto key = std::make_tuple(r, S, v);
    auto it = cdir.find(key);
    if (it != cdir.end()) return it->second;
    const int i = (int)ctab.size();
    ctab.push_back(cval(r, S, v));
    cdir[key] = i;
    return i;
  }
  std::string kinit(int r, uint32_t S, int v) {
    return "opaque_c(p.jtab, " + std::to_string((cbase + dir(r, S, v)) * 8) + "u)[0]";
  }

  std::string opnd(int ti, int v, int id, uint32_t S, std::vector<double>* ks) const {
    const ProdTree& t = tr(ti);
    if (id < t.items()) {
      const int r = t.item_row[id];
      if (r < 0) return ti == 0 ? "Ro" : (v ? "Cy" : "Cx");
      const uint32_t s = S & rs(r);
      if (v == 0 && s == 0) return "x[" + std::to_string(r) + "]";
      if (!ks || live(r, v)) return cname(r, s, v);
      ks->push_back(cval(r, s, v));
      return "(x[" + std::to_string(r) + "] + @" + std::to_string(ks->size() - 1) + "@)";
    }
    const int i = id - t.items();
    if (ks && !nlive(ti, v, i)) return "(" + node(ti, v, i, S, ks) + ")";
    const char* N = ti == 0 ? "o" : (v ? "py" : "px");
    return N + std::to_string(i) + "_" + std::to_string(S & t.sig[i] & ccm);
  }
  bool nlive(int ti, int v, int i) const { return (tr(ti).node_live[i] >> v) & 1u; }
  std::string nname(int ti, int v, int i, uint32_t S) const {
    const char* N = ti == 0 ? "o" : (v ? "py" : "px");
    return N + std::to_string(i) + "_" + std::to_string(S & tr(ti).sig[i] & ccm);
  }
  uint32_t csig(int ti, int id) const {
    const ProdTree& t = tr(ti);
    return (id < t.items() ? t.item_sig[id] : t.sig[id - t.items()]) & ccm;
  }
  std::string iopnd(int ti, int v, int id, uint32_t S) {
    const ProdTree& t = tr(ti);
    if (id < t.items()) {
      const int r = t.item_row[id];
      if (r < 0) return ti == 0 ? "Ro" : (v ? "Cy" : "Cx");
      const uint32_t s = S & rs(r);
      if (s == 0) return v ? "y[" + std::to_string(r) + "]" : "x[" + std::to_string(r) + "]";
      if (live(r, v)) return cname(r, s, v);
      return "(x[" + std::to_string(r) + "] + " + kinit(r, s, v) + ")";
    }
    const int i = id - t.items();
    if (nlive(ti, v, i)) return nname(ti, v, i, S);
    return "(" + iopnd(ti, v, t.a[i], S) + " * " + iopnd(ti, v, t.b[i], S) + ")";
  }
  std::string top(int ti, int v, uint32_t S) const {
    const ProdTree& t = tr(ti);
    return t.root() < 0 ? std::string() : opnd(ti, v, t.root(), S, nullptr);
  }
  std::string node(int ti, int v, int i, uint32_t S, std::vector<double>* ks) const {
    const ProdTree& t = tr(ti);
    return opnd(ti, v, t.a[i], S, ks) + " * " + opnd(ti, v, t.b[i], S, ks);
  }
  uint32_t inner_root_csig() const { return P.inner_tree.root() < 0 ? 0u : csig(1, P.inner_tree.root()); }
  template <class Op>
  std::string dexpr(Op op) const {
    const ProdTree& t = P.inner_tree;
    const int rt = t.root();
    if (rt < t.items()) return op(0, rt) + " - " + op(1, rt);
    const int i = rt - t.items();
    return "__builtin_fma(" + op(0, t.a[i]) + ", " + op(0, t.b[i]) + ", -" + op(1, rt) + ")";
  }
  std::string dname(uint32_t s) const { return "D" + std::to_string(s & inner_root_csig()); }

  void build_class(int c) {
    std::vector<Stmt>& st = cls_stmts[c];
    std::vector<double>& ks = cls_consts[c];
    const std::vector<int>& rows = c < P.seg_b ? P.touched[c + 1] : P.dyn_rows;
    for (int r : rows)
      for (int v = 0; v < (r < len0 ? 2 : 1); ++v)
        if (live(r, v))
          for (uint32_t S : submasks(rs(r))) {
            if (v == 0 && S == 0) continue;
            ks.push_back(cval(r, S, v));
            st.push_back({cname(r, S, v) + " = x[" + std::to_string(r) + "] + @" + std::to_string(ks.size() - 1) +
                          "@;"});
          }
    auto upd = [&](int ti, int v) {
      const ProdTree& t = tr(ti);
      for (int i = 0; i < t.K(); ++i)
        if (((t.sig[i] >> c) & 1u) && nlive(ti, v, i))
          for (uint32_t S : submasks(t.sig[i] & ccm))
            st.push_back({nname(ti, v, i, S) + " = " + node(ti, v, i, S, &ks) + ";"});
    };
    upd(0, 0);
    if ((P.inner_tree.root_sig() >> c) & 1u) {
      upd(1, 0);
      upd(1, 1);
      for (uint32_t S : submasks(inner_root_csig()))
        st.push_back({dname(S) + " = " +
                      dexpr([&](int v, int id) { return opnd(1, v, id, S, &ks); }) + ";"});
    }
  }

  struct Item {
    std::string text;
    std::vector<int> pieces;
    int step = -1;
  };
  std::vector<std::string> pieces;
  std::map<std::string, int> piece_id;
  int next_step_id = 0;
  int piece(const std::string& load_expr) {
    auto it = piece_id.find(load_expr);
    if (it != piece_id.end()) return it->second;
    pieces.push_back(load_expr);
    return piece_id[load_expr] = (int)pieces.size() - 1;
  }
  static std::string pref(int pc, int e) { return "$" + std::to_string(pc) + ":" + std::to_string(e) + "$"; }

  void step_items(std::vector<Item>& out, const std::string& base, const std::string& off,
                  const std::vector<int>& rows, bool full, int c) {
    auto col_piece = [&](int pc) {
      return piece("((cjdbl8*)(" + base + " + " + off + "))[" + std::to_string(pc) + "]");
    };
    const int sid = next_step_id++;
    for (size_t i = 0; i < rows.size(); ++i) {
      const int vi = full ? rows[i] : (int)i, pc = col_piece(vi / 8);
      out.push_back({"x[" + std::to_string(rows[i]) + "] += " + pref(pc, vi % 8) + ";", {pc}, sid});
    }
    if (c < P.seg_cc) return;
    for (const Stmt& st : cls_stmts[c]) {
      Item it;
      it.step = sid;
      const std::string& t = st.text;
      for (size_t q = 0; q < t.size(); ++q) {
        if (t[q] != '@') {
          it.text += t[q];
          continue;
        }
        const size_t e = t.find('@', q + 1);
        const int idx = std::atoi(t.substr(q + 1, e - q - 1).c_str());
        const int pos = cpos[c][idx];
        const bool fresh = std::getenv("SUP_JIT_FRESHBASE") && std::atoi(std::getenv("SUP_JIT_FRESHBASE"));
        const std::string jb = own_stream[c] && !fresh ? "jt" : "(const char*)opaque_c(p.jtab, 0u)";
        const int pc = piece("((cjdbl8*)(" + jb + " + " + std::to_string((cbase + pos - pos % 8) * 8) + "u))[0]");
        it.text += pref(pc, pos % 8);
        if (std::find(it.pieces.begin(), it.pieces.end(), pc) == it.pieces.end()) it.pieces.push_back(pc);
        q = e;
      }
      out.push_back(std::move(it));
    }
  }

  void emit_items(const std::vector<Item>& items, const char* ind) {
    const int kp = P.seg_kp;
    const bool pf = std::getenv("SUP_JIT_PF") ? std::atoi(std::getenv("SUP_JIT_PF")) != 0 : true;
    if (items.empty()) return;
    std::vector<std::pair<size_t, size_t>> reg;
    std::vector<std::vector<int>> rp;
    auto step_pieces = [&](size_t j, std::vector<int> need) {
      for (size_t k = j; k < items.size() && (items[k].step == items[j].step || items[k].step < 0); ++k)
        for (int pc : items[k].pieces)
          if (std::find(need.begin(), need.end(), pc) == need.end()) need.push_back(pc);
      return need;
    };
    const bool xstep = std::getenv("SUP_JIT_XSTEP") ? std::atoi(std::getenv("SUP_JIT_XSTEP")) != 0 : true;
    for (size_t i = 0; i < items.size();) {
      std::vector<int> pcs;
      size_t j = i;
      for (; j < items.size(); ++j) {
        if (j > i && items[j].step >= 0 && items[j].step != items[j - 1].step &&
            (!xstep || (int)step_pieces(j, pcs).size() > kp))
          break;
        std::vector<int> need = pcs;
        for (int pc : items[j].pieces)
          if (std::find(need.begin(), need.end(), pc) == need.end()) need.push_back(pc);
        if ((int)need.size() > kp && j > i) break;
        pcs = need;
      }
      reg.push_back({i, j});
      rp.push_back(pcs);
      i = j;
    }
    const bool accfloat = std::getenv("SUP_JIT_ACCFLOAT") ? std::atoi(std::getenv("SUP_JIT_ACCFLOAT")) != 0 : true;
    std::vector<std::vector<size_t>> order(reg.size());
    for (size_t r = 0; r < reg.size(); ++r)
      for (size_t i = reg[r].first; i < reg[r].second; ++i) order[r].push_back(i);
    if (accfloat)
      for (size_t r = 0; r + 1 < reg.size(); ++r) {
        std::vector<size_t> tail;
        while (!order[r].empty() && items[order[r].back()].step < 0 && items[order[r].back()].pieces.empty() &&
               order[r].size() > 1) {
          tail.insert(tail.begin(), order[r].back());
          order[r].pop_back();
        }
        if (tail.empty()) continue;
        size_t lead = 0;
        while (lead < order[r + 1].size() && items[order[r + 1][lead]].text.compare(0, 2, "x[") == 0) ++lead;
        if (lead == 0) {
          order[r].insert(order[r].end(), tail.begin(), tail.end());
          continue;
        }
        std::vector<size_t> nx;
        const size_t gap = std::max<size_t>(1, lead / (tail.size() + 1));
        size_t t = 0;
        for (size_t i = 0; i < order[r + 1].size(); ++i) {
          if (i == lead)
            while (t < tail.size()) nx.push_back(tail[t++]);
          nx.push_back(order[r + 1][i]);
          if (i < lead && t < tail.size() && (i + 1) % gap == 0) nx.push_back(tail[t++]);
        }
        while (t < tail.size()) nx.push_back(tail[t++]);
        order[r + 1] = nx;
      }
    auto pname = [&](size_t r, int pc) { return "s" + std::to_string(pc) + "_" + std::to_string(r); };
    auto load = [&](size_t r) {
      for (int pc : rp[r]) o << ind << "  jdbl8 " << pname(r, pc) << " = " << pieces[pc] << ";\n";
    };
    auto pin = [&](size_t r) {
      if (rp[r].empty()) return;
      o << ind << "  asm volatile(\"\" :";
      const size_t np = std::min(rp[r].size(), (size_t)std::max(1, kp));
      for (size_t q = 0; q < np; ++q) o << (q ? ", " : " ") << "\"+s\"(" << pname(r, rp[r][q]) << ")";
      o << ");\n";
    };
    o << ind << "{\n";
    load(0);
    pin(0);
    for (size_t r = 0; r < reg.size(); ++r) {
      if (pf && r + 1 < reg.size()) load(r + 1);
      for (size_t i : order[r]) {
        const std::string& t = items[i].text;
        std::string out;
        for (size_t q = 0; q < t.size(); ++q) {
          if (t[q] != '$') {
            out += t[q];
            continue;
          }
          const size_t colon = t.find(':', q + 1), e = t.find('$', q + 1);
          const int pc = std::atoi(t.substr(q + 1, colon - q - 1).c_str());
          out += pname(r, pc) + "[" + t.substr(colon + 1, e - colon - 1) + "]";
          q = e;
        }
        o << ind << "  " << out << "\n";
      }
      if (r + 1 < reg.size()) {
        if (pf) pin(r + 1);
        o << ind << "  __builtin_amdgcn_sched_barrier(0);\n";
        if (!pf) {
          load(r + 1);
          pin(r + 1);
        }
      }
    }
    o << ind << "}\n";
  }

  std::string accumulate_text(bool neg, uint32_t S) const {
    const std::string D = dname(S), U = top(0, 0, S);
    if (U.empty()) return std::string("acc ") + (neg ? "-= " : "+= ") + D + ";";
    return "acc = __builtin_fma(" + std::string(neg ? "-" : "") + D + ", " + U + ", acc);";
  }

  std::string off_const(int k, int neg) const {
    const int blk = (((int)P.touched[k].size() + 7) & ~7);
    return std::to_string((P.jofs[k] + neg * blk) * 8) + "u";
  }
  std::string off_dyn(int k, const char* negv) const {
    const int blk = (((int)P.touched[k].size() + 7) & ~7);
    return std::to_string(P.jofs[k] * 8) + "u + " + negv + " * " + std::to_string(blk * 8) + "u";
  }

  uint32_t state(unsigned st) const {
    uint32_t S = 0;
    for (int i = 0; i < P.seg_cc; ++i) S |= (((st >> i) ^ (st >> (i + 1))) & 1u) << i;
    return S;
  }

  std::vector<double> tail() const {
    std::vector<double> t = ctab;
    t.resize((t.size() + 7) & ~(size_t)7, 0.0);
    for (size_t c = 0; c < cls_consts.size(); ++c) {
      if (!own_stream[c]) continue;
      t.insert(t.end(), cls_consts[c].begin(), cls_consts[c].end());
      t.resize((t.size() + 7) & ~(size_t)7, 0.0);
    }
    return t;
  }

  static std::vector<int> match_stream(const std::vector<double>& need, const std::vector<double>& pool) {
    std::map<uint64_t, std::vector<int>> where;
    for (size_t i = 0; i < pool.size(); ++i) {
      uint64_t k;
      std::memcpy(&k, &pool[i], 8);
      where[k].push_back((int)i);
    }
    std::vector<int> at;
    int prev = -1;
    for (double v : need) {
      uint64_t k;
      std::memcpy(&k, &v, 8);
      auto it = where.find(k);
      if (it == where.end()) return {};
      const std::vector<int>& w = it->second;
      auto nx = std::upper_bound(w.begin(), w.end(), prev);
      prev = nx != w.end() ? *nx : w.front();
      at.push_back(prev);
    }
    return at;
  }
  static int piece_runs(const std::vector<int>& pos) {
    int runs = 0, last = -1;
    for (int p : pos)
      if (p / 8 != last) ++runs, last = p / 8;
    return runs;
  }
  void share_streams(std::vector<int>& host) const {
    const int b = P.seg_b;
    std::vector<int> order;
    for (int c = 0; c <= b; ++c)
      if (!cls_consts[c].empty()) order.push_back(c);
    std::stable_sort(order.begin(), order.end(),
                     [&](int x, int y) { return cls_consts[x].size() > cls_consts[y].size(); });
    for (size_t i = 1; i < order.size(); ++i) {
      const int c = order[i];
      for (size_t j = 0; j < i; ++j) {
        const int h = order[j];
        if (host[h] >= 0) continue;
        const std::vector<int> at = match_stream(cls_consts[c], cls_consts[h]);
        if (at.empty()) continue;
        std::vector<int> own(cls_consts[c].size());
        for (size_t q = 0; q < own.size(); ++q) own[q] = (int)q;
        bool forward = true;
        for (size_t q = 1; q < at.size() && forward; ++q) forward = at[q] / 8 >= at[q - 1] / 8;
        if (forward && 8 * piece_runs(at) <= 9 * piece_runs(own)) {
          host[c] = h;
          break;
        }
      }
    }
  }

  std::string source() {
    const int n = P.n, L = P.lay.L, m = P.lay.m, b = P.seg_b, cc = P.seg_cc;
    const unsigned B = 1u << b, Q = 1u << (m - 1 - b);
    cbase = P.seg_cbase;
    for (int r = 0; r < n; ++r)
      for (int v = 0; v < (r < len0 ? 2 : 1); ++v)
        for (uint32_t S : submasks(rs(r)))
          if (v == 1 || S != 0) dir(r, S, v);
    cls_stmts.assign(b + 1, {});
    cls_consts.assign(b + 1, {});
    for (int c = cc; c <= b; ++c) build_class(c);
    kofs.assign(b + 1, 0);
    own_stream.assign(b + 1, 1);
    std::vector<int> host(b + 1, -1);
    if (!std::getenv("SUP_JIT_NOSHARE")) share_streams(host);
    {
      size_t off = (ctab.size() + 7) & ~(size_t)7;
      for (int c = 0; c <= b; ++c) {
        if (host[c] >= 0) {
          own_stream[c] = 0;
          continue;
        }
        kofs[c] = (int)off;
        off = (off + cls_consts[c].size() + 7) & ~(size_t)7;
      }
    }
    cpos.assign(b + 1, {});
    for (int c = 0; c <= b; ++c) {
      if (host[c] < 0) {
        for (size_t i = 0; i < cls_consts[c].size(); ++i) cpos[c].push_back(kofs[c] + (int)i);
      } else {
        const std::vector<int> at = match_stream(cls_consts[c], cls_consts[host[c]]);
        for (int i : at) cpos[c].push_back(kofs[host[c]] + i);
      }
    }
    if (std::getenv("SUP_JIT_VERBOSE")) {
      std::fprintf(stderr, "  constant streams (doubles): directory %zu", ctab.size());
      for (int c = 0; c <= b; ++c) {
        int same = -1;
        for (int c2 = 0; c2 < c && same < 0; ++c2)
          if (!cls_consts[c].empty() && cls_consts[c2] == cls_consts[c]) same = c2;
        std::vector<double> u = cls_consts[c];
        std::sort(u.begin(), u.end());
        const size_t nd = (size_t)(std::unique(u.begin(), u.end()) - u.begin());
        size_t shared = 0;
        for (double v : cls_consts[c]) {
          bool f = false;
          for (int c2 = 0; c2 < c && !f; ++c2)
            f = std::find(cls_consts[c2].begin(), cls_consts[c2].end(), v) != cls_consts[c2].end();
          shared += f;
        }
        std::fprintf(stderr, ", class %d: %zu (%zu distinct, %zu in earlier streams)%s%s", c, cls_consts[c].size(), nd,
                     shared, same >= 0 ? " (= earlier)" : "", own_stream[c] ? "" : " [reads another class's stream]");
      }
      std::fprintf(stderr, "\n");
    }
    int nlive = 0;
    for (int r = 0; r < n; ++r)
      for (int v = 0; v < 2; ++v) nlive += live(r, v);
    o << "// generated by superman_amd jit.cpp: paired segmented Gray walk, n=" << n << " L=" << L << " m=" << m
      << " segment0=" << len0 << " (" << P.inner_tree.K() << " tree nodes) outer tree nodes=" << P.outer_tree.K()
      << " pair bits specialised=" << b << " cached=" << cc << " live values~" << P.seg_regs
      << " live row-copy sets=" << nlive << "\n";
    o << "#include \"walk_common.hpp\"\n";
    o << "namespace sup {\n";
    o << "typedef double jdbl8 __attribute__((ext_vector_type(8)));\n";
    o << "typedef const __attribute__((address_space(4))) jdbl8 cjdbl8;\n";
    int waves = P.seg_regs <= 64 ? 4 : (P.seg_regs <= kRegs3 ? 3 : 2);
    if (const char* e = std::getenv("SUP_JIT_WAVES")) waves = std::max(1, std::min(8, std::atoi(e)));
    o << "extern \"C\" __global__ __launch_bounds__(kBlock) __attribute__((amdgpu_waves_per_eu(" << waves
      << "))) void sup_walk_seg(WalkParams p) {\n";
    o << "  constexpr int N = " << n << ";\n";
    o << "#define SUP_LANE() ({ uint32_t l_; asm volatile(\"v_mbcnt_lo_u32_b32 %0, -1, 0\\n\\tv_mbcnt_hi_u32_b32 %0, -1, %0\" : \"=v\"(l_)); l_; })\n";
    if (const char* e = std::getenv("SUP_JIT_PHASE"))
      if (std::atoi(e) > 0)
        o << "  if (blockIdx.x & 1u) __builtin_amdgcn_s_sleep(" << std::min(127, std::atoi(e)) << ");\n";
    if (const char* e = std::getenv("SUP_JIT_PRIO"))
      if (std::atoi(e) > 0) o << "  if (blockIdx.x & 1u) __builtin_amdgcn_s_setprio(" << std::min(3, std::atoi(e)) << ");\n";
    o << "  __shared__ double s_keep[" << kBlock / 64 << "][64];\n";
    o << "  __shared__ uint32_t s_vkeep[" << kBlock / 64 << "][64];\n";
    o << "  const uint32_t wv = __builtin_amdgcn_readfirstlane(threadIdx.x >> 6);\n";
    const bool trace = std::getenv("SUP_JIT_TRACE") != nullptr;
    if (trace)
      o << "  const uint64_t tr_r0 = __builtin_amdgcn_s_memrealtime(), tr_c0 = __builtin_amdgcn_s_memtime();\n"
        << "  uint64_t tr_n = 0, tr_sc = 0;\n";
    o << "  for (uint32_t t = next_chunk(p.counter);; t = next_chunk(p.counter)) {\n";
    o << "    const bool head = t < p.tail_ticket;\n";
    o << "    const uint64_t base = head ? (uint64_t)t * p.group\n";
    o << "                               : p.tail_begin + (uint64_t)(t - p.tail_ticket) * p.tail_group;\n";
    o << "    const uint32_t len = head ? p.group : p.tail_group;\n";
    o << "    if (base >= p.chunk_count) break;\n";
    o << "    for (uint32_t j = 0; j < len; ++j) {\n";
    o << "      const uint64_t a = base + j;\n";
    o << "      if (a >= p.chunk_count) break;\n";
    o << "      const uint64_t ga = p.chunk_begin + a;\n";
    o << "      double x[N], y[" << len0 << "];\n";
    if (trace) o << "      const uint64_t tr_s = __builtin_amdgcn_s_memtime();\n";
    o << "      chunk_start" << (P.start_tab_on ? "_tab" : "") << "<N>(x, p, ga, SUP_LANE());\n";
    o << "      {\n";
    o << "        cjdbl8* cv = (cjdbl8*)opaque_c(p.jtab, " << off_const(0, 0) << ");\n";
    for (int r = 0; r < len0; ++r) o << "        y[" << r << "] = x[" << r << "] + cv[" << r / 8 << "][" << r % 8 << "];\n";
    o << "      }\n";
    for (int r = 0; r < n; ++r)
      for (int v = 0; v < (r < len0 ? 2 : 1); ++v)
        if (live(r, v))
          for (uint32_t S : submasks(rs(r))) {
            if (S == 0) continue;
            o << "      double " << cname(r, S, v) << " = x[" << r << "] + " << kinit(r, S, v) << ";\n";
          }
    auto tree_init = [&](int ti, int v) {
      const ProdTree& t = tr(ti);
      if (t.tail_hi > t.tail_lo)
        o << "      const double " << (ti == 0 ? "Ro" : (v ? "Cy" : "Cx")) << " = "
          << tree(t.tail_lo, t.tail_hi, v ? "y" : "x") << ";\n";
      for (int i = 0; i < t.K(); ++i)
        if (this->nlive(ti, v, i))
          for (uint32_t S : submasks(t.sig[i] & ccm))
            o << "      double " << nname(ti, v, i, S) << " = " << iopnd(ti, v, t.a[i], S) << " * "
              << iopnd(ti, v, t.b[i], S) << ";\n";
    };
    tree_init(0, 0);
    o << "      double acc = 0.0;\n";
    o << "      uint32_t vis = 0;\n";
    if (P.outer_tree.tail_hi > P.outer_tree.tail_lo)
      o << "      if (__builtin_amdgcn_ballot_w64(SUP_LANE() < " << (1u << L) << "u && Ro != 0.0) != 0) {\n";
    else
      o << "      {\n";
    o << "      vis = " << (1u << m) << "u;\n";
    tree_init(1, 0);
    tree_init(1, 1);
    if (P.inner_tree.root() >= 0)
      for (uint32_t S : submasks(inner_root_csig()))
        o << "      double " << dname(S) << " = " << dexpr([&](int v, int id) { return iopnd(1, v, id, S); })
          << ";\n";
    else
      o << "      double D0 = 0.0;\n";
    {
      const std::string U = top(0, 0, 0);
      o << "      acc = " << (U.empty() ? dname(0) : dname(0) + " * " + U) << ";\n";
    }
    o << "      double tot = 0.0;\n";
    if (trace) o << "      asm volatile(\"\" : \"+v\"(acc));\n      tr_sc += __builtin_amdgcn_s_memtime() - tr_s;\n      ++tr_n;\n";
    o << "      for (uint32_t q = 0; q < " << Q << "u; ++q) {\n";
    const char* ind = "        ";
    o << ind << "const char* jt = (const char*)opaque_c(p.jtab, 0u);\n";
    o << ind << "const uint32_t ng = q & 1u;\n";
    {
      std::vector<Item> items;
      for (unsigned st = 1; st < B; ++st) {
        const int pb = __builtin_ctz(st), k = pb + 1;
        if (pb >= cc && !P.touched[k].empty())
          step_items(items, "jt", pb < b - 1 ? off_const(k, (st >> (pb + 1)) & 1u) : off_dyn(k, "ng"),
                     P.touched[k], false, step_class(k, b));
        items.push_back({accumulate_text(st & 1u, state(st)), {}});
      }
      emit_items(items, ind);
    }
    if (Q > 1) {
      o << ind << "if (q + 1u < " << Q << "u) {\n";
      o << ind << "  const uint32_t kk = (uint32_t)__builtin_ctz(q + 1u);\n";
      o << ind << "  const uint32_t ngd = ((q + 1u) >> (kk + 1u)) & 1u;\n";
      {
        std::vector<Item> items;
        step_items(items, "(const char*)opaque_c(p.cols, 0u)",
                   "(2u * (" + std::to_string(L + b + 1) + "u + kk) + ngd) * " + std::to_string(P.NP * 8) + "u",
                   P.dyn_rows, true, P.seg_b);
        items.push_back({accumulate_text(false, 0u), {}});
        emit_items(items, "          ");
      }
      o << ind << "  tot += acc;\n" << ind << "  acc = 0.0;\n";
      o << ind << "}\n";
    }
    o << "      }\n";
    o << "      acc = tot + acc;\n";
    o << "      if (((uint32_t)ga ^ (uint32_t)__builtin_popcount(SUP_LANE())) & 1u) acc = -acc;\n";
    o << "      }\n";
    o << "      const uint32_t lane = SUP_LANE();\n";
    o << "      const double part = wave_sum(lane < " << (1u << L) << "u ? acc : 0.0);\n";
    o << "      if (lane == j) s_keep[wv][j] = part, s_vkeep[wv][j] = vis;\n";
    o << "    }\n";
    o << "    __builtin_amdgcn_fence(__ATOMIC_RELEASE, \"wavefront\");\n";
    o << "    __builtin_amdgcn_wave_barrier();\n";
    o << "    __builtin_amdgcn_fence(__ATOMIC_ACQUIRE, \"wavefront\");\n";
    o << "    const uint32_t lane = SUP_LANE();\n";
    o << "    chunk_store(base, len, s_keep[wv][lane], s_vkeep[wv][lane]);\n";
    o << "    __builtin_amdgcn_wave_barrier();\n";
    o << "  }\n";
    if (trace)
      o << "  if (p.trace && SUP_LANE() == 0) {\n"
        << "    unsigned long long* t = p.trace + 8ull * (blockIdx.x * " << kBlock / 64 << "u + wv);\n"
        << "    t[0] = tr_r0; t[1] = __builtin_amdgcn_s_memrealtime(); t[2] = tr_c0;\n"
        << "    t[3] = __builtin_amdgcn_s_memtime(); t[4] = tr_n; t[5] = tr_sc;\n"
        << "  }\n";
    o << "}\n";
    o << "}  // namespace sup\n";
    return o.str();
  }
};

const char* const kJitOpts[] = {"--offload-arch=gfx950", "-O3", "-std=c++17", "-ffp-contract=off"};
constexpr int kJitNopts = 4;

}

std::vector<std::string> jit_opts() {
  std::vector<std::string> v(kJitOpts, kJitOpts + kJitNopts);
  if (const char* e = std::getenv("SUP_JIT_SCHED"))
    if (*e) v.push_back("-mllvm"), v.push_back(std::string("-amdgpu-sched-strategy=") + e);
  if (const char* e = std::getenv("SUP_JIT_OPAQUE_R2"))
    if (std::atoi(e)) v.push_back("-DSUP_OPAQUE_BEFORE_OFFSET=1");
  return v;
}

namespace {

uint64_t fnv1a(const std::string& s, uint64_t h = 1469598103934665603ull) {
  for (unsigned char c : s) h = (h ^ c) * 1099511628211ull;
  return h;
}

std::string hiprtc_version() {
  static const std::string v = [] {
    int major = 0, minor = 0;
    if (hiprtcVersion(&major, &minor) != HIPRTC_SUCCESS) return std::string("hiprtc ?");
    std::string r = "hiprtc " + std::to_string(major) + "." + std::to_string(minor) + " hip " + std::to_string(HIP_VERSION);
    Dl_info di;
    if (dladdr(reinterpret_cast<void*>(&hiprtcCreateProgram), &di) && di.dli_fname) {
      const char* slash = std::strrchr(di.dli_fname, '/');
      r += std::string(" ") + (slash ? slash + 1 : di.dli_fname);
      std::ifstream f(di.dli_fname, std::ios::binary);
      if (f) {
        std::string bytes((std::istreambuf_iterator<char>(f)), std::istreambuf_iterator<char>());
        char hx[40];
        std::snprintf(hx, sizeof hx, " %zu %016llx", bytes.size(), (unsigned long long)fnv1a(bytes));
        r += hx;
      }
    }
    return r;
  }();
  return v;
}

}

uint64_t toolchain_hash_impl() {
  std::string key;
  for (const std::string& opt : jit_opts()) key += "\n//" + opt;
  key += std::string("\n//") + kWalkCommonSrc + kWalkParamsSrc;
  key += "\n//" + hiprtc_version();
  return fnv1a(key);
}

namespace {

uint64_t jit_source_key(const std::string& src) {
  std::string key = src;
  for (const std::string& opt : jit_opts()) key += "\n//" + opt;
  key += std::string("\n//") + kWalkCommonSrc + kWalkParamsSrc;
  key += "\n//" + hiprtc_version();
  return fnv1a(key);
}

}

constexpr size_t kStartTabMaxBytes = 16u << 20;
constexpr int kStartTabMaxWalkBits = 12;

static void seg_start_table(Plan& P) {
  const int n = P.n, NP = P.NP;
  const uint64_t C = P.lay.chunks();
  const unsigned hb = (unsigned)(P.lay.L + P.lay.m);
  P.start_tab.assign((size_t)C * NP, 0.0);
  const size_t blocks = (size_t)std::min<uint64_t>(C, 64);
  parallel_tasks(blocks, [&](size_t b) {
    for (uint64_t ga = C * b / blocks; ga < C * (b + 1) / blocks; ++ga) {
      double* x = P.start_tab.data() + (size_t)ga * NP;
      for (int j = 0; j < NP; ++j) x[j] = P.x0[j];
      for (uint64_t h = ga ^ (ga >> 1); h; h &= h - 1) {
        const double* col = P.cols.data() + (size_t)(2u * (hb + (unsigned)__builtin_ctzll(h))) * NP;
        for (int j = 0; j < n; ++j) x[j] += col[j];
      }
    }
  });
}

int build_seg(Plan& P, int fixed_budget) {
  const int n = P.n, L = P.lay.L, m = P.lay.m;
  if (m < 3) {
    set_error("segmented walk needs >= 3 walk bits");
    return SUP_EINVAL;
  }
  if (P.cols.empty()) return SUP_EINVAL;
  P.start_tab.clear();
  P.start_tab_on = !std::getenv("SUP_JIT_NO_START_TAB") && P.lay.m <= kStartTabMaxWalkBits &&
                   (double)P.lay.chunks() * P.NP * sizeof(double) <= (double)kStartTabMaxBytes;
  P.touched.assign(m, {});
  P.seg_start.assign(1, 0);
  std::vector<char> seen(n, 0);
  int R = 0;
  for (int k = 0; k < m; ++k) {
    const double* col = P.cols.data() + (size_t)(2 * (L + k)) * P.NP;
    for (int j = 0; j < n; ++j)
      if (col[j] != 0.0) {
        P.touched[k].push_back(j);
        if (!seen[j]) seen[j] = 1, ++R;
      }
    if (R > P.seg_start.back()) P.seg_start.push_back(R);
  }
  for (int j = 0; j < R; ++j)
    if (!seen[j]) {
      set_error("segmented walk: rows are not in first-touch order");
      return SUP_EINVAL;
    }
  if (P.touched[0].empty()) {
    set_error("segmented walk: walk column 0 has no nonzero");
    return SUP_EINVAL;
  }
  {
    const int len0 = P.seg_start[1];
    std::vector<char> got(len0, 0);
    int cnt = 0;
    P.sub_start.assign(1, 0);
    for (int k = 1; k < m; ++k) {
      for (int r : P.touched[k])
        if (r < len0 && !got[r]) {
          if (r != cnt) {
            set_error("segmented walk: segment 0 rows are not in sub-segment order");
            return SUP_EINVAL;
          }
          got[r] = 1, ++cnt;
        }
      if (cnt > P.sub_start.back()) P.sub_start.push_back(cnt);
    }
  }
  if (P.seg_b < 1 || P.seg_b > m - 1) {
    P.seg_b = seg_static_bits(m);
    if (!std::getenv("SUP_JIT_B")) {
      double best = 1e300;
      for (const int cb : seg_b_candidates(m)) {
        SegRows R;
        R.n = n, R.m = m, R.touched = P.touched;
        R.len0 = P.seg_start[1], R.s_end = P.sub_start.back(), R.r_end = P.seg_start.back();
        seg_rows_finish(R, cb);
        const SegFit f = seg_best(R, std::min(max_cached(), P.lay.cc_cap));
        const double sc = seg_block_bytes(f, cb) > kMaxBlockBytes ? 1e300 : seg_score(f);
        if (sc < best - 1e-12) best = sc, P.seg_b = cb;
      }
    }
  }
  P.dyn_rows.clear();
  {
    std::vector<char> in(n, 0);
    for (int k = P.seg_b + 1; k < m; ++k)
      for (int r : P.touched[k]) in[r] = 1;
    for (int j = 0; j < n; ++j)
      if (in[j]) P.dyn_rows.push_back(j);
  }
  SegRows SR;
  SR.n = n, SR.m = m, SR.touched = P.touched;
  SR.len0 = P.seg_start[1], SR.s_end = P.sub_start.back(), SR.r_end = P.seg_start.back();
  seg_rows_finish(SR, P.seg_b);
  const int cc_cap = std::min(max_cached(), P.lay.cc_cap);
  auto finish = [&SR, &cc_cap, n, L, m](Plan& Q, int budget) {
    SegFit f;
    if (const char* e = std::getenv("SUP_JIT_CC"))
      f = seg_fit(SR, std::max(0, std::min({std::atoi(e), SR.b - 1, kMaxCachedBits})), budget);
    else f = seg_best(SR, cc_cap, budget);
    if (const char* e = std::getenv("SUP_JIT_STORAGE")) f = seg_fit(SR, f.cc, std::max(0, std::atoi(e)));
    Q.outer_tree = std::move(f.outer);
    Q.inner_tree = std::move(f.inner);
    Q.seg_cc = f.cc;
    Q.seg_ops = f.ops;
    Q.seg_regs = f.regs;
    Q.seg_budget = budget;
    Q.jofs.assign(m, 0);
    Q.jtab.clear();
    for (int k = 0; k < m; ++k) {
      const std::vector<int>& t = Q.touched[k];
      const size_t blk = (t.size() + 7) & ~(size_t)7;
      Q.jofs[k] = (int)Q.jtab.size();
      Q.jtab.resize(Q.jtab.size() + 2 * std::max<size_t>(blk, 8), 0.0);
      for (size_t i = 0; i < t.size(); ++i) {
        Q.jtab[Q.jofs[k] + i] = Q.cols[(size_t)(2 * (L + k)) * Q.NP + t[i]];
        Q.jtab[Q.jofs[k] + blk + i] = Q.cols[(size_t)(2 * (L + k) + 1) * Q.NP + t[i]];
      }
    }
    Q.seg_cbase = Q.jtab.size();
    Q.seg_kp = 4;
    if (const char* e = std::getenv("SUP_JIT_KP")) Q.seg_kp = std::max(1, std::atoi(e));
    Gen g(Q);
    Q.jit_src = g.source();
    {
      const std::vector<double> t = g.tail();
      Q.jtab.insert(Q.jtab.end(), t.begin(), t.end());
    }
    Q.jit_key = jit_source_key(Q.jit_src);
    (void)n;
  };
  const char* env_budget = std::getenv("SUP_JIT_BUDGET");
  if (env_budget) fixed_budget = std::max(1, std::atoi(env_budget));
  finish(P, fixed_budget > 0 ? fixed_budget : kRegsMax);
  const bool fixed = fixed_budget > 0 || std::getenv("SUP_JIT_REGMAX") || std::getenv("SUP_JIT_STORAGE") ||
                     std::getenv("SUP_JIT_CC") || std::getenv("SUP_JIT_NOVERIFY");
  const double walk_s = std::ldexp(1.0, n - 1) * P.seg_ops / 3.7e13;
  if (fixed && std::getenv("SUP_JIT_VERBOSE")) {
    CodeScan s;
    const int rc = jit_code_scan(P, &s);
    std::fprintf(stderr, "  fixed budget %d: ops %.4f rc %d vgprs %d spills %d scratch %dB (loop %d of %d insts)\n",
                 P.seg_budget, P.seg_ops, rc, s.vgprs, s.vgpr_spills, s.scratch_bytes, s.loop_scratch, s.loop_insts);
  }
  if (!fixed && walk_s < 0.01 && P.seg_cc > 3) {
    CodeScan s;
    P.seg_loop_scratch = jit_code_scan(P, &s) != SUP_OK || s.loop_scratch != 0;
  }
  if (!fixed && walk_s >= 0.01 && P.seg_regs > kRegs3) {
    std::vector<int> budgets;
    for (int b2 = kRegs3 + 20; b2 <= kRegsMax + 60; b2 += 8) budgets.push_back(b2);
    std::vector<Plan> cand(budgets.size(), P);
    parallel_tasks(budgets.size(), [&](size_t i) { finish(cand[i], budgets[i]); });
    std::vector<size_t> idx;
    for (size_t i = 0; i < cand.size(); ++i) {
      bool dup = false;
      for (size_t j : idx) dup = dup || cand[j].jit_key == cand[i].jit_key;
      if (!dup) idx.push_back(i);
    }
    std::vector<CodeScan> scans(cand.size());
    std::vector<int> src(cand.size(), SUP_EHIP);
    std::vector<char> done(cand.size(), 0);
    auto compile_one = [&](size_t i) {
      if (done[i]) return;
      const auto t0 = std::chrono::steady_clock::now();
      const double own = t_compile_ms;
      src[i] = jit_code_scan(cand[i], &scans[i]);
      t_compile_ms = own + std::chrono::duration<double, std::milli>(std::chrono::steady_clock::now() - t0).count();
      done[i] = 1;
    };
    auto clean = [&](size_t i) { return done[i] && src[i] == SUP_OK && scans[i].loop_scratch == 0; };
    size_t pp = 0;
    for (size_t k = 0; k < idx.size(); ++k)
      if (budgets[idx[k]] <= kRegsMax) pp = k;
    enum { kUnknown = 0, kFail, kDirty, kCleanScratch, kClean0 };
    constexpr long kLadderDone = -1, kLadderFail = -2;
    auto next_needed = [&](const std::vector<int>& o) -> long {
      const size_t probe = idx[pp];
      if (o[probe] == kUnknown) return (long)probe;
      if (o[probe] == kFail) return kLadderFail;
      auto cl = [&](size_t i) { return o[i] >= kCleanScratch; };
      size_t c_pos;
      if (cl(probe)) {
        size_t lo = pp, hi = idx.size();
        while (hi - lo > 1) {
          const size_t mid = lo + (hi - lo) / 2;
          if (o[idx[mid]] == kUnknown) return (long)idx[mid];
          (cl(idx[mid]) ? lo : hi) = mid;
        }
        c_pos = lo;
      } else {
        long lo = -1, hi = (long)pp;
        while (hi - lo > 1) {
          const long mid = lo + (hi - lo) / 2;
          if (o[idx[mid]] == kUnknown) return (long)idx[mid];
          (cl(idx[mid]) ? lo : hi) = mid;
        }
        if (lo < 0) return kLadderFail;
        c_pos = (size_t)lo;
      }
      if (o[idx[c_pos]] != kClean0)
        for (size_t k = c_pos; k-- > 0;) {
          if (cand[idx[k]].seg_ops > cand[idx[c_pos]].seg_ops * (1.0 + kScratchTolerance)) break;
          if (o[idx[k]] == kUnknown) return (long)idx[k];
          if (o[idx[k]] == kClean0) break;
        }
      return kLadderDone;
    };
    std::vector<int> outcome(cand.size(), kUnknown);
    const size_t procs = rtc_procs();
    for (;;) {
      const long k = next_needed(outcome);
      if (k < 0) break;
      if (procs > 1 && !jit_code_cached(cand[k])) {
        std::vector<const Plan*> batch;
        std::vector<char> queued(cand.size(), 0);
        std::queue<std::vector<int>> q;
        q.push(outcome);
        for (size_t visits = 0; !q.empty() && batch.size() < procs && visits < 4096; ++visits) {
          std::vector<int> h = std::move(q.front());
          q.pop();
          const long s = next_needed(h);
          if (s < 0) continue;
          if (!queued[s] && !jit_code_cached(cand[s])) queued[s] = 1, batch.push_back(&cand[s]);
          for (int r : {kDirty, kCleanScratch, kClean0}) {
            std::vector<int> h2 = h;
            h2[s] = r;
            q.push(std::move(h2));
          }
        }
        const auto t0 = std::chrono::steady_clock::now();
        prefetch_compiles(batch, procs);
        t_compile_ms += std::chrono::duration<double, std::milli>(std::chrono::steady_clock::now() - t0).count();
      }
      compile_one((size_t)k);
      outcome[k] = src[k] != SUP_OK         ? kFail
                   : scans[k].loop_scratch  ? kDirty
                   : scans[k].scratch_bytes ? kCleanScratch
                                            : kClean0;
    }
    if (outcome[idx[pp]] == kFail) return SUP_EHIP;
    auto pick = [&]() {
      int c = -1, bare = -1;
      for (size_t i : idx) {
        if (!clean(i)) continue;
        if (c < 0 || cand[i].seg_ops < cand[c].seg_ops) c = (int)i;
        if (scans[i].scratch_bytes == 0 && (bare < 0 || cand[i].seg_ops < cand[bare].seg_ops)) bare = (int)i;
      }
      return (bare >= 0 && c >= 0 && cand[bare].seg_ops <= cand[c].seg_ops * (1.0 + kScratchTolerance)) ? bare : c;
    };
    const int best = pick();
    if (std::getenv("SUP_JIT_VERBOSE"))
      for (size_t i : idx)
        if (done[i])
          std::fprintf(stderr, "  budget %d: ops %.4f rc %d vgprs %d spills %d scratch %dB (loop %d of %d insts, %d readlane)%s\n",
                       budgets[i], cand[i].seg_ops, src[i], scans[i].vgprs, scans[i].vgpr_spills,
                       scans[i].scratch_bytes, scans[i].loop_scratch, scans[i].loop_insts, scans[i].loop_readlane,
                       (int)i == best ? "  <- chosen" : "");
    if (best < 0) {
      set_error("segmented walk: every budget's kernel touches scratch inside its walk loop (or fails to compile)");
      return SUP_EHIP;
    }
    P = std::move(cand[best]);
  }
  P.seg_skip = seg_skip_fraction_plan(P, 2048);
  if (P.start_tab_on) seg_start_table(P);
  if (std::getenv("SUP_JIT_VERBOSE"))
    std::fprintf(stderr, "seg plan n=%d m=%d b=%d ops/step=%.4f regs=%d cc=%d table=%zu B (columns %zu B) key=%016llx "
                 "(storage plans evaluated: %ld)\n", n, m, P.seg_b, P.seg_ops, P.seg_regs, P.seg_cc,
                 P.jtab.size() * sizeof(double), P.seg_cbase * sizeof(double), (unsigned long long)P.jit_key,
                 g_fit_calls.load());
  return SUP_OK;
}

std::string seg_source(const Plan& P, int kp) {
  Plan Q = P;
  Q.seg_kp = kp;
  return Gen(Q).source();
}

}
```

### superman_amd/csrc/jit_compile.cpp

```cpp
#include <dlfcn.h>
#include <hip/hip_runtime.h>
#include <hip/hiprtc.h>
#include <sched.h>
#include <signal.h>
#include <spawn.h>
#include <sys/stat.h>
#include <sys/wait.h>
#include <unistd.h>

#include <algorithm>
#include <atomic>
#include <cerrno>
#include <chrono>
#include <condition_variable>
#include <cstdio>
#include <cstdlib>
#include <cstring>
#include <fstream>
#include <map>
#include <memory>
#include <mutex>
#include <sstream>
#include <string>
#include <thread>
// ... 244 lines not shown
        pid_t pid = 0;
        if (posix_spawn(&pid, helper.c_str(), nullptr, nullptr, argv.data(), environ) != 0) continue;
        int status = 0;
        const auto t_spawn = std::chrono::steady_clock::now();
        bool done = false;
        for (;;) {
          const pid_t w = ::waitpid(pid, &status, WNOHANG);
          if (w == pid) {
            done = true;
            break;
          }
          if (w < 0 && errno != EINTR) break;
          if (std::chrono::steady_clock::now() - t_spawn > std::chrono::seconds(kHelperLimitS)) {
            ::kill(pid, SIGKILL);
            while (::waitpid(pid, &status, 0) < 0 && errno == EINTR) {
            }
            break;
          }
          ::usleep(1000);
        }
        if (!done || !WIFEXITED(status) || WEXITSTATUS(status) != 0) continue;
        auto co = std::make_shared<std::vector<char>>();
        if (!read_file(dir + "/" + name + ".co", *co)) continue;
        {
          std::lock_guard<std::mutex> g(g_jit_mu);
          g_code.emplace(P.jit_key, co);
        }
        const std::string cdir = cache_dir();
        if (!cdir.empty()) write_file_atomic(cdir, name + ".co", *co);
      }
    };
    std::vector<std::thread> th;
    for (size_t t = 0; t < std::min(procs, todo.size()); ++t) th.emplace_back(worker);
    for (auto& t : th) t.join();
  }
  for (const std::string& f : made) ::unlink((dir + "/" + f).c_str());
  ::rmdir(dir.c_str());
}

namespace {

int resolve(int dev, const Plan& P, hipFunction_t* fn) {
  if (P.kind != kWalkSeg || P.jit_src.empty()) {
    set_error("plan has no segmented-walk kernel");
    return SUP_EINVAL;
  }
  auto k = std::make_pair(dev, P.jit_key);
  {
    std::lock_guard<std::mutex> g(g_jit_mu);
    auto it = g_fn.find(k);
    if (it != g_fn.end()) {
      *fn = it->second;
      return SUP_OK;
    }
  }
  std::shared_ptr<std::vector<char>> code;
  int rc = compile(P, code);
  if (rc) return rc;
  std::lock_guard<std::mutex> g(g_jit_mu);
  auto it = g_fn.find(k);
  if (it != g_fn.end()) {
    *fn = it->second;
    return SUP_OK;
  }
  hipModule_t mod;
  hipError_t e = hipModuleLoadData(&mod, code->data());
  if (e != hipSuccess) {
    set_error(std::string("hipModuleLoadData (segmented walk): ") + hipGetErrorString(e));
    return SUP_EHIP;
  }
  if ((e = hipModuleGetFunction(fn, mod, "sup_walk_seg")) != hipSuccess) {
    set_error(std::string("hipModuleGetFunction (segmented walk): ") + hipGetErrorString(e));
    return SUP_EHIP;
  }
  g_fn[k] = *fn;
  return SUP_OK;
}

}

int jit_compile_only(const Plan& P, double* compile_ms) {
  if (P.kind != kWalkSeg || P.jit_src.empty()) {
    set_error("plan has no segmented-walk kernel");
    return SUP_EINVAL;
  }
  const double before = jit_compile_ms_thread();
  std::shared_ptr<std::vector<char>> code;
  const int rc = compile(P, code);
  if (compile_ms) *compile_ms = jit_compile_ms_thread() - before;
  return rc;
}

int jit_code_scan(const Plan& P, CodeScan* out) {
  std::shared_ptr<std::vector<char>> code;
  const int rc = compile(P, code);
  if (rc) return rc;
  return scan_code_object(*code, "sup_walk_seg", out);
}

int jit_occupancy(int dev, const Plan& P, int* blocks_per_cu, double* compile_ms) {
  const double before = jit_compile_ms_thread();
  hipFunction_t fn;
  int rc = resolve(dev, P, &fn);
  if (rc) return rc;
  if (compile_ms) *compile_ms = jit_compile_ms_thread() - before;
  std::lock_guard<std::mutex> g(g_jit_mu);
  auto k = std::make_pair(dev, P.jit_key);
  auto it = g_occ.find(k);
  if (it != g_occ.end()) {
    *blocks_per_cu = it->second;
    return SUP_OK;
  }
  int b = 0;
  hipError_t e = hipModuleOccupancyMaxActiveBlocksPerMultiprocessor(&b, fn, kBlock, jit_lds_bytes());
  if (e != hipSuccess) {
    set_error(std::string("occupancy query (segmented walk): ") + hipGetErrorString(e));
    return SUP_EHIP;
  }
  g_occ[k] = b > 0 ? b : 1;
  *blocks_per_cu = g_occ[k];
  return SUP_OK;
}

int jit_launch(int dev, const Plan& P, const WalkParams& p, int grid, hipStream_t s) {
  hipFunction_t fn;
  int rc = resolve(dev, P, &fn);
  if (rc) return rc;
  WalkParams arg = p;
  void* args[] = {&arg};
  hipError_t e = hipModuleLaunchKernel(fn, (unsigned)grid, 1, 1, kBlock, 1, 1, jit_lds_bytes(), s, args, nullptr);
  if (e != hipSuccess) {
    set_error(std::string("hipModuleLaunchKernel (segmented walk): ") + hipGetErrorString(e));
    return SUP_EHIP;
  }
  return SUP_OK;
}

double jit_compile_ms_thread() { return t_compile_ms; }

uint64_t jit_toolchain_hash() {
  static const uint64_t h = toolchain_hash_impl();
  return h;
}

bool seg_choice_load(uint64_t key, int* m, SegChoice* c) {
  const std::string dir = cache_dir();
  if (dir.empty()) return false;
  std::vector<char> buf;
  if (!read_file(dir + "/plan_" + key_hex(key) + ".txt", buf)) return false;
  buf.push_back('\0');
  std::istringstream in(buf.data());
  std::string tag;
  int ver = 0, cnt = 0;
  if (!(in >> tag >> ver >> *m >> c->b >> c->budget >> c->cc_cap >> cnt) || tag != "supseg" || ver != 3 || cnt < 1 ||
      cnt > 64 || c->cc_cap < 0 || c->cc_cap > kMaxCachedBits)
    return false;
  c->order.resize(cnt);
  for (int& v : c->order)
    if (!(in >> v) || v < 0 || v > 63) return false;
  return true;
}

bool seg_choice_exists(uint64_t key) {
  const std::string dir = cache_dir();
  struct stat sb;
  return !dir.empty() && ::stat((dir + "/plan_" + key_hex(key) + ".txt").c_str(), &sb) == 0;
}

void seg_choice_store(uint64_t key, int m, const SegChoice& c) {
  const std::string dir = cache_dir();
  if (dir.empty() || c.order.empty()) return;
  std::ostringstream o;
  o << "supseg 3 " << m << ' ' << c.b << ' ' << c.budget << ' ' << c.cc_cap << ' ' << c.order.size();
  for (int v : c.order) o << ' ' << v;
  o << '\n';
  const std::string str = o.str();
  write_file_atomic(dir, "plan_" + key_hex(key) + ".txt", std::vector<char>(str.begin(), str.end()));
}

int auto_decision_load(uint64_t key) {
  const std::string dir = cache_dir();
  if (dir.empty()) return -1;
  std::vector<char> buf;
  if (!read_file(dir + "/auto_" + key_hex(key) + ".txt", buf)) return -1;
  buf.push_back('\0');
  std::istringstream in(buf.data());
  std::string tag;
  int ver = 0, v = -1;
  if (!(in >> tag >> ver >> v) || tag != "supauto" || ver != 1 || (v != 0 && v != 1)) return -1;
  return v;
}

int auto_decision_store(uint64_t key, int seg) {
  const std::string dir = cache_dir();
  if (dir.empty()) return seg;
  const std::string name = "auto_" + key_hex(key) + ".txt";
  const std::string str = std::string("supauto 1 ") + (seg ? "1" : "0") + "\n";
  const std::string mine = "." + name + ".new" + std::to_string(::getpid()) + "." +
                           std::to_string(std::hash<std::thread::id>()(std::this_thread::get_id()));
  write_file_atomic(dir, mine, std::vector<char>(str.begin(), str.end()));
  (void)::link((dir + "/" + mine).c_str(), (dir + "/" + name).c_str());
  std::remove((dir + "/" + mine).c_str());
  const int on_disk = auto_decision_load(key);
  return on_disk >= 0 ? on_disk : seg;
}

double seg_cold_model(int n) {
  const double search = 0.39 * std::exp2((n - 40) / 6.5) * std::pow(16.0 / plan_threads(), 0.8);
  return search + 1.25;
}

static std::string seg_cost_name() { return "cost_" + key_hex(jit_toolchain_hash()) + ".txt"; }

double seg_cost_ratio_load() {
  const std::string dir = cache_dir();
  if (dir.empty()) return -1.0;
  std::vector<char> buf;
  if (!read_file(dir + "/" + seg_cost_name(), buf)) return -1.0;
  buf.push_back('\0');
  std::istringstream in(buf.data());
  std::string tag;
  int ver = 0;
  double r = -1.0;
  if (!(in >> tag >> ver >> r) || tag != "supcost" || ver != 2 || !(r > 0.0) || r > 1000.0) return -1.0;
  return r;
}

double seg_cold_predict(int n) {
  const char* e = std::getenv("SUP_JIT_COLD_RATIO");
  const double r = e ? std::atof(e) : seg_cost_ratio_load();
  return seg_cold_model(n) * (r > 0.0 ? std::min(8.0, std::max(0.25, r)) : 1.0);
}

void seg_cost_store(int n, double seconds) {
  const std::string dir = cache_dir();
  if (dir.empty() || !(seconds > 0.0)) return;
  char b[64];
  std::snprintf(b, sizeof b, "supcost 2 %.4f\n", seconds / seg_cold_model(n));
  const std::string str = b;
  write_file_atomic(dir, seg_cost_name(), std::vector<char>(str.begin(), str.end()));
}

}
```

### superman_amd/csrc/plan.cpp

```cpp
#include "engine.hpp"

#include <algorithm>
#include <atomic>
#include <chrono>
#include <cmath>
#include <cstdio>
#include <cstdlib>
#include <cstring>
#include <map>
#include <memory>
#include <mutex>
#include <thread>
#include <tuple>

#include <unistd.h>

namespace sup {

static thread_local std::string g_err;
void set_error(const std::string& msg) { g_err = msg; }
const char* last_error() { return g_err.c_str(); }

bool env_on(const char* name, bool dflt) {
  const char* e = std::getenv(name);
// ... 287 lines not shown
int improve_sparse_plan(const double* A, int n, const Layout& lay, Plan& P) {
  if (P.kind != kWalkSparse || !P.integral || lay.m < 3 ||
      ops_seconds(gray_steps(n), walk_cost(P)) < kChunkEndSearchSec)
    return SUP_OK;
  std::vector<int> base;
  for (int k = 0; k < lay.m; ++k) base.push_back(P.colmap[lay.L + k]);
  for (int e = 0; e < lay.L; ++e) base.push_back(P.colmap[e]);
  SegChoice c;
  if (!skip_walk_order(A, n, lay, c.order, &base, 0.9)) return SUP_OK;
  Plan Q;
  const int rc = make_plan(A, n, kWalkSparse, false, lay, Q, &c);
  if (rc == SUP_OK) P = std::move(Q);
  return rc;
}

double walk_cost(const Plan& P) {
  if (P.kind == kWalkDense) return 2.0 * P.n + 1.0;
  if (P.kind == kWalkSeg) return seg_walk_cost(P);
  double cost = 0.0, w = 0.5;
  for (int k = 0; k < P.lay.m; ++k, w *= 0.5) cost += w * (16.0 * P.nblk[P.lay.L + k] + 1.0);
  return cost + w * 16.0 * ((P.n + 7) / 8);
}

static double walk_cost_eff(const Plan& P) {
  return P.kind == kWalkSeg ? walk_cost(P) * (1.0 - P.seg_skip) : walk_cost(P);
}

double walk_seconds(const Plan& P, double steps) { return ops_seconds(steps, walk_cost_eff(P)); }

static bool no_chunk_ends() { static const bool off = env_on("SUP_NO_CHUNK_ENDS", false); return off; }

int make_plan(const double* A, int n, WalkKind kind, bool identity_map, const Layout& lay, Plan& P,
              const SegChoice* choice) {
  if (n < 1 || n > SUP_MAX_N) {
    set_error("n must be in [1, 64]");
    return SUP_EINVAL;
  }
  P = Plan();
  P.n = n;
  P.NP = pad8(n);
  P.kind = kind;
  P.lay = lay;
  P.integral = is_integral(A, n);
  const int nb = n - 1;
  const int L = lay.L, m = lay.m;

  P.colmap.resize(nb);
  for (int e = 0; e < nb; ++e) P.colmap[e] = e;
  const bool given_order = (kind == kWalkSkip || kind == kWalkDense || kind == kWalkSparse) && choice && m > 0;
  if (!identity_map && (kind == kWalkSparse || kind == kWalkSeg || given_order) && m > 0) {
    int segb = 0;
    std::vector<int> order;
    auto valid_order = [&](const std::vector<int>& o) {
      if ((int)o.size() != m + L) return false;
      std::vector<char> seen(nb, 0);
      for (int v : o) {
        if (v < 0 || v >= nb || seen[v]) return false;
        seen[v] = 1;
      }
      return true;
    };
    if (given_order) {
      if (!valid_order(choice->order)) {
        set_error("walk column order: not m + L distinct flippable columns");
        return SUP_EINVAL;
      }
      order = choice->order;
    } else if (kind == kWalkSeg && choice && valid_order(choice->order) && choice->b >= 0 && choice->b <= m) {
      order = choice->order;
      segb = choice->b;
    } else {
      order = kind == kWalkSeg ? seg_walk_order(A, n, m, m + L, &segb, lay.cc_cap) : greedy_walk_order(A, n, m + L);
    }
    P.seg_b = segb;
    if (kind == kWalkSeg) P.seg_order.assign(order.begin(), order.begin() + (m + L));
    std::vector<char> used(n, 0);
    for (int k = 0; k < m; ++k) P.colmap[L + k] = order[k], used[order[k]] = 1;
    for (int e = 0; e < L; ++e) P.colmap[e] = order[m + e], used[order[m + e]] = 1;
    int e = L + m;
    std::vector<char> top(n, 0);
    if (kind == kWalkSeg || given_order) {
      std::vector<char> wrow(n, 0);
      for (int k = 0; k < (given_order ? m + L : m); ++k)
        for (int i = 0; i < n; ++i) wrow[i] |= A[(size_t)i * n + order[k]] != 0.0;
      for (int c = 0; c < nb && P.integral; ++c) {
        top[c] = 1;
        for (int i = 0; i < n; ++i)
          if (!wrow[i] && A[(size_t)i * n + c] != 0.0) top[c] = 0;
      }
    }
    for (int pass = 0; pass < 2; ++pass)
      for (int c = 0; c < nb; ++c)
        if (!used[c] && top[c] == pass) P.colmap[e++] = c;
  }

  P.rowperm.resize(n);
  for (int j = 0; j < n; ++j) P.rowperm[j] = j;
  P.nblk.assign(std::max(nb, 1), 0);
  P.rowmask.assign(n, 0);
  if (kind != kWalkDense) {
    std::vector<char> placed(n, 0);
    std::vector<int> order;
    order.reserve(n);
    for (int k = 0; k < m; ++k) {
      const int c = P.colmap[L + k];
      for (int i = 0; i < n; ++i)
        if (!placed[i] && A[(size_t)i * n + c] != 0.0) {
          placed[i] = 1;
          order.push_back(i);
        }
      P.nblk[L + k] = ((int)order.size() + 7) / 8;
    }
    for (int i = 0; i < n; ++i)
      if (!placed[i]) order.push_back(i);
    P.rowperm = order;
    if (kind == kWalkSeg) {
      std::vector<int> walk(m);
      for (int k = 0; k < m; ++k) walk[k] = P.colmap[L + k];
      P.rowperm = seg_row_order(A, n, walk);
    }
  }
  for (int e = 0; e < nb; ++e)
    if (e < L || e >= L + m) P.nblk[e] = (n + 7) / 8;

  P.cols.assign((size_t)2 * std::max(nb, 1) * P.NP, 0.0);
  for (int e = 0; e < nb; ++e) {
    const int c = P.colmap[e];
    for (int j = 0; j < n; ++j) {
      const double v = A[(size_t)P.rowperm[j] * n + c];
      P.cols[(size_t)(2 * e) * P.NP + j] = v;
      P.cols[(size_t)(2 * e + 1) * P.NP + j] = -v;
    }
  }
  std::vector<double> x0(n);
  double p0;
  nw_start(A, n, x0.data(), &p0);
  P.x0.assign(P.NP, 0.0);
  for (int j = 0; j < n; ++j) P.x0[j] = x0[P.rowperm[j]];

  P.umask = 0;
  for (int j = 0; j < n; ++j) {
    const int i = P.rowperm[j];
    bool lane_touched = false;
    for (int e = 0; e < L; ++e)
      if (A[(size_t)i * n + P.colmap[e]] != 0.0) lane_touched = true;
    if (!lane_touched) P.umask |= 1ull << j;
    uint64_t rm = 0;
    for (int k = 0; k < m; ++k)
      if (A[(size_t)i * n + P.colmap[L + k]] != 0.0) rm |= 1ull << k;
    P.rowmask[j] = rm;
    if ((kind == kWalkSparse || kind == kWalkDense) && !lane_touched && rm == 0 && !no_chunk_ends())
      P.chunk_ends |= 1ull << j;
  }
  if (kind == kWalkSeg) return build_seg(P, choice ? choice->budget : 0);
  return SUP_OK;
}

static constexpr double kJitMinSavingSec = 3.0;
static constexpr double kAutoRuns = 4.0;
static constexpr double kJitWarmSavingSec = 0.1;
static constexpr int kJitWarmMinN = 30;

static int plan_for_uncached(const double* A, int n, sup_kernel kernel, const Layout& lay, Plan& P, int jit,
                             int ndev, int dev, double min_saving);
static double auto_min_saving(const double* A, int n, const Layout& lay, int jit);

static constexpr double kSegStartOps = 2048.0;

static constexpr int kSegMinChunkBits = 14;

static uint64_t knob_hash() {
  Fnv1a f;
  for (char** e = environ; e && *e; ++e) {
    const char* v = *e;
    if (std::strncmp(v, "SUP_JIT_", 8) != 0 || !std::strncmp(v, "SUP_JIT_CACHE_DIR=", 18) ||
        !std::strncmp(v, "SUP_JIT_DUMP=", 13) || !std::strncmp(v, "SUP_JIT_VERBOSE=", 16) ||
        !std::strncmp(v, "SUP_JIT_COLD_RATIO=", 19))
      continue;
    f.bytes(v, std::strlen(v));
    f.bytes("\xff", 1);
  }
  return f.h;
}

static uint64_t seg_disk_key(const double* A, int n, const Layout& lay) {
  Fnv1a f{0x5eed5e9a11ull ^ jit_toolchain_hash()};
  const size_t nn = (size_t)n * n;
  const bool integral = is_integral(A, n);
  const int32_t head[] = {6 , n, lay.L, lay.m, (int32_t)lay.fixed, (int32_t)integral};
  f.bytes(head, sizeof head);
  if (integral) {
    f.bytes(A, nn * sizeof(double));
  } else {
    std::vector<unsigned char> pat((nn + 7) / 8, 0);
    for (size_t i = 0; i < nn; ++i)
      if (A[i] != 0.0) pat[i / 8] |= (unsigned char)(1u << (i % 8));
    f.bytes(pat.data(), pat.size());
  }
  const uint64_t k = knob_hash();
  f.bytes(&k, sizeof k);
  return f.h;
}

static int make_seg_plan(const double* A, int n, const Layout& lay, Plan& P) {
  const uint64_t dkey = seg_disk_key(A, n, lay);
  {
    int m2 = 0;
    SegChoice c;
    if (seg_choice_load(dkey, &m2, &c) && m2 >= 3 && m2 <= lay.m + lay.h && (!lay.fixed || m2 == lay.m)) {
      Layout l2 = lay;
      l2.m = m2;
      l2.h = lay.m + lay.h - m2;
      l2.cc_cap = c.cc_cap;
      if (make_plan(A, n, kWalkSeg, false, l2, P, &c) == SUP_OK) return SUP_OK;
    }
  }
  const auto t_cold = std::chrono::steady_clock::now();
  auto plan = [A, n](const Layout& l, Plan& Q) {
    int r = make_plan(A, n, kWalkSeg, false, l, Q);
    if (r == SUP_OK && Q.seg_loop_scratch && l.cc_cap > 3) {
      Layout l3 = l;
      l3.cc_cap = 3;
      r = make_plan(A, n, kWalkSeg, false, l3, Q);
    }
    return r;
  };
  int rc = plan(lay, P);
  if (rc) return rc;
  if (!lay.fixed) {
    const int mmax = std::min(lay.m + lay.h - kSegMinChunkBits, 31);
    int m2 = lay.m;
    while (m2 < mmax && std::ldexp(walk_cost(P), m2) < 32.0 * kSegStartOps) ++m2;
    if (m2 != lay.m) {
      Layout l2 = lay;
      l2.m = m2;
      l2.h = lay.m + lay.h - m2;
      Plan s2;
      if (plan(l2, s2) == SUP_OK) {
        auto eff = [](const Plan& q) {
          return (1.0 - q.seg_skip) * (walk_cost(q) + std::ldexp(kSegStartOps, -q.lay.m));
        };
        if (eff(s2) < eff(P)) P = std::move(s2);
      }
    }
  }
  SegChoice c;
  c.order = P.seg_order;
  c.b = P.seg_b;
  c.budget = P.seg_budget;
  c.cc_cap = P.lay.cc_cap;
  seg_choice_store(dkey, P.lay.m, c);
  const double cold_s = std::chrono::duration<double>(std::chrono::steady_clock::now() - t_cold).count();
  seg_cost_store(n, cold_s);
  if (std::getenv("SUP_JIT_VERBOSE"))
    std::fprintf(stderr, "cold segmented plan n=%d: %.3f s (compiles %.3f s wall on this thread)\n", n, cold_s,
                 jit_compile_ms_thread() * 1e-3);
  return SUP_OK;
}

namespace {
struct PlanKey {
  uint64_t hash;
  int n, kernel, L, m, jit, ndev;
  bool fixed;
  uint64_t knobs;
  bool operator<(const PlanKey& o) const {
    return std::tie(hash, n, kernel, L, m, jit, ndev, fixed, knobs) <
           std::tie(o.hash, o.n, o.kernel, o.L, o.m, o.jit, o.ndev, o.fixed, o.knobs);
  }
};
std::mutex g_plan_mu;
std::map<PlanKey, std::pair<std::vector<double>, std::shared_ptr<const Plan>>> g_plans;
constexpr size_t kPlanCacheMax = 32;
}

int plan_for_shared(const double* A, int n, sup_kernel kernel, const Layout& lay, std::shared_ptr<const Plan>& out,
                    int jit, int ndev, int dev, bool keep) {
  const size_t nn = (size_t)n * n;
  uint64_t l[4] = {1469598103934665603ull, 0x9e3779b97f4a7c15ull, 0xc2b2ae3d27d4eb4full, 0x165667b19e3779f9ull};
  size_t i = 0;
  for (; i + 4 <= nn; i += 4)
    for (int k = 0; k < 4; ++k) {
      uint64_t b;
      std::memcpy(&b, A + i + k, 8);
      l[k] = (l[k] ^ b) * 1099511628211ull;
    }
  for (; i < nn; ++i) {
    uint64_t b;
    std::memcpy(&b, A + i, 8);
    l[0] = (l[0] ^ b) * 1099511628211ull;
  }
  uint64_t h = l[0];
  for (int k = 1; k < 4; ++k) h = (h ^ l[k]) * 1099511628211ull;
  const PlanKey key{h, n, (int)kernel, lay.L, lay.m, jit, jit == 0 ? ndev : 0, lay.fixed, knob_hash()};
  auto cached = [&]() {
    auto it = g_plans.find(key);
    if (it == g_plans.end() || !std::equal(A, A + nn, it->second.first.begin())) return false;
    out = it->second.second;
    return true;
  };
  {
    std::lock_guard<std::mutex> g(g_plan_mu);
    if (cached()) return SUP_OK;
  }
  auto P = std::make_shared<Plan>();
  const int rc = plan_for_uncached(A, n, kernel, lay, *P, jit, ndev, dev, auto_min_saving(A, n, lay, jit));
  if (rc) return rc;
  if (!keep) {
    out = P;
    return SUP_OK;
  }
  std::lock_guard<std::mutex> g(g_plan_mu);
  if (cached()) return SUP_OK;
  if (g_plans.size() >= kPlanCacheMax) g_plans.clear();
  static uint64_t next_uid = 0;
  P->uid = ++next_uid;
  out = P;
  g_plans[key] = {std::vector<double>(A, A + nn), out};
  return SUP_OK;
}

int plan_for(const double* A, int n, sup_kernel kernel, const Layout& lay, Plan& P, int jit, int ndev, int dev) {
  std::shared_ptr<const Plan> sp;
  const int rc = plan_for_shared(A, n, kernel, lay, sp, jit, ndev, dev);
  if (rc == SUP_OK) P = *sp;
  return rc;
}

static constexpr double kSkipEfficiency = 0.62;
static constexpr double kSkipPriceEfficiency = 0.90;
static constexpr double kSkipSearchMinSec = 4.0;

static double skip_visited_fraction(const Plan& P, int dev) {
  int nd = 0;
  if (device_count(&nd) != SUP_OK || nd < 1) return -1.0;
  if (dev < 0 || dev >= nd) dev = 0;
  const uint64_t C = P.lay.chunks(), len = std::max<uint64_t>(1, C / 512);
  uint64_t vis = 0, tot = 0;
  for (uint64_t i = 0; i < 8; ++i) {
    uint64_t c0 = (2 * i + 1) * C / 16;
    if (c0 + len > C) c0 = C - len;
    RangeResult r;
    if (run_range(dev, P, c0, c0 + len, true, r) != SUP_OK) return -1.0;
    vis += r.visited;
    tot += len << (P.lay.L + P.lay.m);
  }
  return tot ? (double)vis / (double)tot : 1.0;
}

static double auto_min_saving(const double* A, int n, const Layout& lay, int jit) {
  if (jit != 0 || n < kJitWarmMinN) return kJitMinSavingSec;
  if (seg_choice_exists(seg_disk_key(A, n, lay))) return kJitWarmSavingSec;
  return std::max(kJitWarmSavingSec, seg_cold_predict(n) / kAutoRuns);
}

struct AutoRecord {
  uint64_t key = 0;
  int recorded = -1;
  bool active = false;
  AutoRecord(const double* A, int n, const Layout& lay, sup_kernel kernel, int ndev, int jit, double walk_s) {
    active = jit == 0 && n >= kJitWarmMinN && walk_s >= kJitWarmSavingSec;
    if (!active) return;
    key = seg_disk_key(A, n, lay) ^ (0x9e3779b97f4a7c15ull * (uint64_t)(1 + (int)kernel)) ^
          ((uint64_t)std::max(ndev, 1) << 48);
    recorded = auto_decision_load(key);
  }
  bool store(bool seg) const {
    if (active && recorded < 0) return auto_decision_store(key, seg ? 1 : 0) == 1;
    return seg;
  }
};

static int plan_for_uncached(const double* A, int n, sup_kernel kernel, const Layout& lay, Plan& P, int jit,
                             int ndev, int dev, double min_saving) {
  std::vector<WalkKind> kinds;
  auto make_seg = [&](Plan& s) { return make_seg_plan(A, n, lay, s); };
  switch (kernel) {
    case SUP_KERNEL_SKIPPER: {
      int rc = make_plan(A, n, kWalkSkip, false, lay, P);
      if (rc) return rc;
      const bool integral = P.integral;
      if (integral && n >= 10 &&
          ops_seconds(gray_steps(n), walk_cost(P), kSkipEfficiency * kLaneOpsPerSec) >= kSkipSearchMinSec) {
        SegChoice c;
        Plan Q;
        if (skip_walk_order(A, n, lay, c.order, nullptr, 0.5) && make_plan(A, n, kWalkSkip, false, lay, Q, &c) == SUP_OK)
          P = std::move(Q);
      }
      if (jit < 0 || n < 10 || lay.m < 3) return SUP_OK;
      const double steps = gray_steps(n, ndev);
      double skip_cost = walk_cost(P) / (integral ? kSkipPriceEfficiency : 1.0);
      const AutoRecord rec(A, n, lay, kernel, ndev, jit, ops_seconds(steps, skip_cost));
      if (rec.recorded == 0) return SUP_OK;
      Plan s;
      if (rec.recorded == 1) {
        if (make_seg(s) == SUP_OK) P = std::move(s);
        return SUP_OK;
      }
      auto decide = [&]() -> bool {
        if (jit < 1 && ops_seconds(steps, skip_cost) < min_saving) return false;
        if (make_seg(s) != SUP_OK) return false;
        if (walk_cost_eff(s) >= skip_cost) return false;
// ... 94 lines not shown
```

Baseline: 3155 billion gray-steps/s.

## Unroll high Gray-code bit steps into JIT segmented walk with op-census selection

Adds a JIT code path that unrolls up to three higher Gray-code bits beyond the segment width into the generated walk loop. The emitted code recomputes only the statements that depend on rows touched by each step, and shared steps are hoisted out. A per-step fp64 op census counts the work, and the planner compares candidate hi values and register-budget ladders against the plain plan to pick the cheaper one. It also exposes the census through a new C/Python API and bumps the ABI and cache format. The risks are larger generated code and register pressure, plus roughly double the compile work during planning.

```diff
diff --git a/include/superman.h b/include/superman.h
--- a/include/superman.h
+++ b/include/superman.h
@@ -8,7 +8,7 @@
 extern "C" {
 #endif
 
-#define SUP_ABI_VERSION 15
+#define SUP_ABI_VERSION 16
 
 #define SUP_OK            0
 #define SUP_EINVAL      (-1)
@@ -102,6 +102,10 @@
 int sup_plan_info(const void* mat, sup_dtype t, int n, sup_kernel kernel, const sup_opts* o, int* walk_kind,
                   int* colmap, int* lane_bits, int* walk_bits, int* cached_bits, int* pair_bits,
                   double* est_ops_per_step);
+
+#define SUP_CENSUS_CLASSES 14
+int sup_plan_census(const void* mat, sup_dtype t, int n, sup_kernel kernel, const sup_opts* o, int* hi_bits,
+                    double* census);
 
 int sup_plan_key(const void* mat, sup_dtype t, int n, sup_kernel kernel, const sup_opts* o, uint64_t* key);
 
diff --git a/superman_amd/__init__.py b/superman_amd/__init__.py
--- a/superman_amd/__init__.py
+++ b/superman_amd/__init__.py
@@ -10,7 +10,7 @@
                    SCHED_STATIC, SupApproxResult, SupError, SupOpts, SupReduceOpts, SupStats)
 
 __all__ = [
-    "perman", "perman_cpu", "perman_exact", "perman_exact_range", "perman_quad", "perman_quad_range", "perman_complex", "perman_complex_range", "perman_complex_batch", "perman_complex_submatrices", "perman_complex_fock", "perman_complex_fock_plan", "perman_complex_minors", "perman_complex_minors_submatrices", "perman_complex_minors_range", "boson_sample", "read_mtx_complex", "partial", "perman_shard", "plan_info", "plan_key", "prepare", "read_matrix", "read_mtx", "sort_order",
+    "perman", "perman_cpu", "perman_exact", "perman_exact_range", "perman_quad", "perman_quad_range", "perman_complex", "perman_complex_range", "perman_complex_batch", "perman_complex_submatrices", "perman_complex_fock", "perman_complex_fock_plan", "perman_complex_minors", "perman_complex_minors_submatrices", "perman_complex_minors_range", "boson_sample", "read_mtx_complex", "partial", "perman_shard", "plan_info", "plan_census", "CENSUS_CLASSES", "plan_key", "prepare", "read_matrix", "read_mtx", "sort_order",
     "skip_order", "compress", "decompose", "perman_reduced", "approx", "grid_graph", "ALGOS_APPROX",
     "nw_start", "device_count", "rccl_devices", "layout", "ShardCall", "SupError", "ALGOS_DENSE", "ALGOS_SPARSE",
     "gpu_perman64_xshared_coalescing_mshared",
@@ -499,6 +499,23 @@
             "cached": cc.value, "pair_bits": pb.value, "est_ops_per_step": ops.value}
 
 
+CENSUS_CLASSES = ("x_adds", "copy_adds", "outer_forms", "inner_forms", "d_fmas", "accumulates", "lane_sum",
+                  "shared_adds", "shared_copies", "shared_forms", "hi_adds", "hi_copies", "hi_forms")
+
+
+def plan_census(mat, kernel: str = "dense", jit: int = 0, gpu_num: int = 1, device_id: int = 0,
+                walk_log2: int = 0) -> dict:
+    a, dt, n = _mat(mat)
+    lib = _lib.load()
+    hi = C.c_int()
+    cen = np.zeros(len(CENSUS_CLASSES) + 1, np.float64)
+    o = _opts(gpu_num=gpu_num, device_id=device_id, jit=jit, walk_log2=walk_log2)
+    _lib.check(lib.sup_plan_census(a.ctypes.data, dt, n, _KERNELS[kernel], C.byref(o), C.byref(hi), cen.ctypes.data),
+               "plan_census")
+    return {"hi_bits": hi.value, "classes": dict(zip(CENSUS_CLASSES, (float(v) for v in cen))),
+            "chunk_start": float(cen[-1])}
+
+
 def plan_key(mat, kernel: str = "dense", jit: int = 0, gpu_num: int = 1, device_id: int = 0,
              walk_log2: int = 0) -> int:
     a, dt, n = _mat(mat)
diff --git a/superman_amd/_lib.py b/superman_amd/_lib.py
--- a/superman_amd/_lib.py
+++ b/superman_amd/_lib.py
@@ -26,7 +26,7 @@
 
 EXPORTS = [
     "sup_opts_init", "sup_abi_version", "sup_last_error", "sup_device_count", "sup_rccl_devices", "sup_device_checks", "sup_device_warmup", "sup_kernel_time",
-    "sup_perman", "sup_partial", "sup_perman_cpu", "sup_nw_start", "sup_perman_shard", "sup_plan_info",
+    "sup_perman", "sup_partial", "sup_perman_cpu", "sup_nw_start", "sup_perman_shard", "sup_plan_info", "sup_plan_census",
     "sup_prepare", "sup_plan_key", "sup_perman_exact", "sup_perman_exact_range", "sup_perman_reduced_exact",
     "sup_perman_quad", "sup_perman_quad_range",
     "sup_perman_reduced_quad", "sup_perman_complex", "sup_perman_complex_range", "sup_read_mtx_complex",
@@ -124,7 +124,7 @@
             build()
         lib = C.CDLL(LIB_PATH)
         _declare(lib)
-        if lib.sup_abi_version() != 15:
+        if lib.sup_abi_version() != 16:
             raise RuntimeError("libsuperman_hip.so ABI version mismatch")
         _lib = lib
         return lib
@@ -171,6 +171,7 @@
     lib.sup_perman_shard.argtypes = [P, I, I, I, I, I, C.POINTER(SupOpts), C.POINTER(D), C.POINTER(SupStats)]
     lib.sup_plan_info.argtypes = [P, I, I, I, C.POINTER(SupOpts), C.POINTER(I), P, C.POINTER(I), C.POINTER(I),
                                   C.POINTER(I), C.POINTER(I), C.POINTER(D)]
+    lib.sup_plan_census.argtypes = [P, I, I, I, C.POINTER(SupOpts), C.POINTER(I), P]
     lib.sup_prepare.argtypes = [P, I, I, I, C.POINTER(SupOpts), C.POINTER(I), C.POINTER(C.c_double)]
     lib.sup_plan_key.argtypes = [P, I, I, I, C.POINTER(SupOpts), C.POINTER(C.c_uint64)]
     lib.sup_nw_start.argtypes = [P, I, I, C.POINTER(D), C.POINTER(D)]
diff --git a/superman_amd/csrc/capi.cpp b/superman_amd/csrc/capi.cpp
--- a/superman_amd/csrc/capi.cpp
+++ b/superman_amd/csrc/capi.cpp
@@ -637,6 +637,26 @@
     for (int e = 0; e < n - 1; ++e) colmap[e] = P.colmap[e];
   if (L) *L = P.lay.L;
   if (m) *m = P.lay.m;
+  return SUP_OK;
+}
+
+static_assert(SUP_CENSUS_CLASSES == kSegCensusN, "superman.h lists the census classes of engine.hpp");
+
+int sup_plan_census(const void* mat, sup_dtype t, int n, sup_kernel kernel, const sup_opts* o_in, int* hi_bits,
+                    double* census) {
+  std::vector<double> A;
+  int rc = to_double(mat, t, n, A);
+  if (rc) return rc;
+  sup_opts o;
+  if (o_in) o = *o_in;
+  else sup_opts_init(&o);
+  Plan P;
+  if ((rc = check_walk_opts(o))) return rc;
+  if ((rc = plan_for(A.data(), n, kernel, layout_for(n, o), P, o.jit, o.gpu_num, o.device_id))) return rc;
+  const bool seg = P.kind == kWalkSeg;
+  if (hi_bits) *hi_bits = seg ? P.seg_hi : 0;
+  if (census)
+    for (int c = 0; c < kSegCensusN; ++c) census[c] = seg ? P.seg_census[c] : 0.0;
   return SUP_OK;
 }
 
diff --git a/superman_amd/csrc/engine.hpp b/superman_amd/csrc/engine.hpp
--- a/superman_amd/csrc/engine.hpp
+++ b/superman_amd/csrc/engine.hpp
@@ -21,6 +21,24 @@
 void nw_start(const double* A, int n, double* x0, double* p0);
 
 constexpr int kMaxCachedBits = 4;
+
+enum SegCensus {
+  kCenXAdd = 0,
+  kCenCopy,
+  kCenOuter,
+  kCenInner,
+  kCenD,
+  kCenAcc,
+  kCenLane,
+  kCenSharedAdd,
+  kCenSharedCopy,
+  kCenSharedForm,
+  kCenHiAdd,
+  kCenHiCopy,
+  kCenHiForm,
+  kCenStart,
+  kSegCensusN
+};
 
 struct Layout {
   int L;
@@ -70,6 +88,9 @@
   bool integral = false;
   int seg_cc = 0;
   double seg_ops = 0.0;
+  double seg_model_ops = 0.0;
+  int seg_hi = 0;
+  double seg_census[kSegCensusN] = {};
   double seg_skip = 0.0;
   int seg_regs = 0;
   int seg_budget = 0;
@@ -91,6 +112,7 @@
   int b = 0;
   int budget = 0;
   int cc_cap = kMaxCachedBits;
+  int hi = 0;
 };
 
 int make_plan(const double* A, int n, WalkKind kind, bool identity_map, const Layout& lay, Plan& P,
@@ -106,7 +128,7 @@
 double seg_skip_estimate(const double* A, int n, const std::vector<int>& order, int m, int samples);
 double seg_skip_fraction_plan(const Plan& P, int samples);
 std::vector<int> seg_row_order(const double* A, int n, const std::vector<int>& walk);
-int build_seg(Plan& P, int fixed_budget = 0);
+int build_seg(Plan& P, int fixed_budget = 0, int fixed_hi = 0);
 bool seg_choice_load(uint64_t key, int* m, SegChoice* c);
 bool seg_choice_exists(uint64_t key);
 double seg_cold_model(int n);
diff --git a/superman_amd/csrc/jit.cpp b/superman_amd/csrc/jit.cpp
--- a/superman_amd/csrc/jit.cpp
+++ b/superman_amd/csrc/jit.cpp
@@ -737,7 +737,16 @@
 
 struct Stmt {
   std::string text;
+  int row = -1, ti = -1, node = -1;
+  bool isD = false;
+  int adds = 0, muls = 0, dops = 0;
 };
+
+int count_sub(const std::string& t, const char* pat) {
+  int c = 0;
+  for (size_t q = t.find(pat); q != std::string::npos; q = t.find(pat, q + 1)) ++c;
+  return c;
+}
 
 struct Gen {
   const Plan& P;
@@ -857,34 +866,68 @@
           for (uint32_t S : submasks(rs(r))) {
             if (v == 0 && S == 0) continue;
             ks.push_back(cval(r, S, v));
-            st.push_back({cname(r, S, v) + " = x[" + std::to_string(r) + "] + @" + std::to_string(ks.size() - 1) +
-                          "@;"});
+            Stmt s{cname(r, S, v) + " = x[" + std::to_string(r) + "] + @" + std::to_string(ks.size() - 1) + "@;"};
+            s.row = r, s.adds = 1;
+            st.push_back(std::move(s));
           }
     auto upd = [&](int ti, int v) {
       const ProdTree& t = tr(ti);
       for (int i = 0; i < t.K(); ++i)
         if (((t.sig[i] >> c) & 1u) && nlive(ti, v, i))
-          for (uint32_t S : submasks(t.sig[i] & ccm))
-            st.push_back({nname(ti, v, i, S) + " = " + node(ti, v, i, S, &ks) + ";"});
+          for (uint32_t S : submasks(t.sig[i] & ccm)) {
+            Stmt s{nname(ti, v, i, S) + " = " + node(ti, v, i, S, &ks) + ";"};
+            s.ti = ti, s.node = i, s.adds = count_sub(s.text, " + @"), s.muls = count_sub(s.text, " * ");
+            st.push_back(std::move(s));
+          }
     };
     upd(0, 0);
     if ((P.inner_tree.root_sig() >> c) & 1u) {
       upd(1, 0);
       upd(1, 1);
-      for (uint32_t S : submasks(inner_root_csig()))
-        st.push_back({dname(S) + " = " +
-                      dexpr([&](int v, int id) { return opnd(1, v, id, S, &ks); }) + ";"});
-    }
+      for (uint32_t S : submasks(inner_root_csig())) {
+        Stmt s{dname(S) + " = " + dexpr([&](int v, int id) { return opnd(1, v, id, S, &ks); }) + ";"};
+        s.ti = 1, s.isD = true, s.dops = 1;
+        s.adds = count_sub(s.text, " + @"), s.muls = count_sub(s.text, " * ");
+        st.push_back(std::move(s));
+      }
+    }
+  }
+
+  std::vector<Stmt> stmts_for(const std::vector<int>& rows) const {
+    std::vector<char> in(P.n, 0);
+    for (int r : rows) in[r] = 1;
+    std::vector<char> hit[2];
+    for (int ti = 0; ti < 2; ++ti) {
+      const ProdTree& t = tr(ti);
+      hit[ti].assign(t.items() + t.K(), 0);
+      for (int j = 0; j < t.items(); ++j) hit[ti][j] = t.item_row[j] >= 0 && in[t.item_row[j]];
+      for (int i = 0; i < t.K(); ++i) hit[ti][t.items() + i] = hit[ti][t.a[i]] || hit[ti][t.b[i]];
+    }
+    std::vector<Stmt> out;
+    for (const Stmt& s : cls_stmts[P.seg_b]) {
+      const bool need = s.row >= 0   ? (bool)in[s.row]
+                        : s.isD      ? P.inner_tree.root() >= 0 && hit[1][P.inner_tree.root()]
+                        : s.node >= 0 ? (bool)hit[s.ti][tr(s.ti).items() + s.node]
+                                      : true;
+      if (need) out.push_back(s);
+    }
+    return out;
   }
 
   struct Item {
     std::string text;
     std::vector<int> pieces;
     int step = -1;
+    std::string decl;
   };
+  std::string step_base;
   std::vector<std::string> pieces;
   std::map<std::string, int> piece_id;
   int next_step_id = 0;
+  double body[kSegCensusN] = {};
+  double census[kSegCensusN] = {};
+  double block_bytes = 0.0;
+  enum StepMode { kPairStep = 0, kSharedStep = 1, kHiStep = 2 };
   int piece(const std::string& load_expr) {
     auto it = piece_id.find(load_expr);
     if (it != piece_id.end()) return it->second;
@@ -894,7 +937,10 @@
   static std::string pref(int pc, int e) { return "$" + std::to_string(pc) + ":" + std::to_string(e) + "$"; }
 
   void step_items(std::vector<Item>& out, const std::string& base, const std::string& off,
-                  const std::vector<int>& rows, bool full, int c) {
+                  const std::vector<int>& rows, bool full, int c, StepMode mode = kPairStep,
+                  const std::vector<Stmt>* stmts = nullptr) {
+    const int cen_add = mode == kPairStep ? kCenXAdd : (mode == kSharedStep ? kCenSharedAdd : kCenHiAdd);
+    const int cen_copy = mode == kPairStep ? kCenCopy : (mode == kSharedStep ? kCenSharedCopy : kCenHiCopy);
     auto col_piece = [&](int pc) {
       return piece("((cjdbl8*)(" + base + " + " + off + "))[" + std::to_string(pc) + "]");
     };
@@ -902,9 +948,17 @@
     for (size_t i = 0; i < rows.size(); ++i) {
       const int vi = full ? rows[i] : (int)i, pc = col_piece(vi / 8);
       out.push_back({"x[" + std::to_string(rows[i]) + "] += " + pref(pc, vi % 8) + ";", {pc}, sid});
+      body[cen_add] += 1.0;
     }
     if (c < P.seg_cc) return;
-    for (const Stmt& st : cls_stmts[c]) {
+    for (const Stmt& st : stmts ? *stmts : cls_stmts[c]) {
+      body[cen_copy] += st.adds;
+      if (mode == kPairStep) {
+        body[st.ti == 0 ? kCenOuter : kCenInner] += st.muls;
+        body[kCenD] += st.dops;
+      } else {
+        body[mode == kSharedStep ? kCenSharedForm : kCenHiForm] += st.muls + st.dops;
+      }
       Item it;
       it.step = sid;
       const std::string& t = st.text;
@@ -917,7 +971,8 @@
         const int idx = std::atoi(t.substr(q + 1, e - q - 1).c_str());
         const int pos = cpos[c][idx];
         const bool fresh = std::getenv("SUP_JIT_FRESHBASE") && std::atoi(std::getenv("SUP_JIT_FRESHBASE"));
-        const std::string jb = own_stream[c] && !fresh ? "jt" : "(const char*)opaque_c(p.jtab, 0u)";
+        const std::string jb = own_stream[c] && !fresh ? (step_base.empty() ? std::string("jt") : step_base)
+                                                       : std::string("(const char*)opaque_c(p.jtab, 0u)");
         const int pc = piece("((cjdbl8*)(" + jb + " + " + std::to_string((cbase + pos - pos % 8) * 8) + "u))[0]");
         it.text += pref(pc, pos % 8);
         if (std::find(it.pieces.begin(), it.pieces.end(), pc) == it.pieces.end()) it.pieces.push_back(pc);
@@ -990,6 +1045,8 @@
       }
     auto pname = [&](size_t r, int pc) { return "s" + std::to_string(pc) + "_" + std::to_string(r); };
     auto load = [&](size_t r) {
+      for (size_t i = reg[r].first; i < reg[r].second; ++i)
+        if (!items[i].decl.empty()) o << ind << "  " << items[i].decl << "\n";
       for (int pc : rp[r]) o << ind << "  jdbl8 " << pname(r, pc) << " = " << pieces[pc] << ";\n";
     };
     auto pin = [&](size_t r) {
@@ -1114,6 +1171,76 @@
         }
       }
     }
+  }
+
+  void hi_loop(unsigned Q, unsigned U, int u) {
+    const int L = P.lay.L, m = P.lay.m, b = P.seg_b, cc = P.seg_cc;
+    const unsigned B = 1u << b;
+    o << "      for (uint32_t qq = 0; qq < " << Q / U << "u; ++qq) {\n";
+    const char* ind = "        ";
+    o << ind << "const uint32_t ngh = qq & 1u;\n";
+    for (unsigned i = 0; i < U; ++i) {
+      o << ind << "{\n";
+      std::vector<Item> items;
+      auto own_base = [&](size_t first) {
+        if (items.size() > first)
+          items[first].decl = "const char* " + step_base + " = (const char*)opaque_c(p.jtab, 0u);";
+        step_base.clear();
+      };
+      for (unsigned st = 1; st < B; ++st) {
+        const int pb = __builtin_ctz(st), k = pb + 1;
+        if (pb >= cc && !P.touched[k].empty()) {
+          const size_t first = items.size();
+          step_base = "jt" + std::to_string(next_step_id);
+          step_items(items, step_base, off_const(k, pb < b - 1 ? (st >> (pb + 1)) & 1u : i & 1u), P.touched[k],
+                     false, step_class(k, b));
+          own_base(first);
+        }
+        items.push_back({accumulate_text(st & 1u, state(st)), {}});
+        body[kCenAcc] += 1.0;
+      }
+      if (i + 1 < U) {
+        const int kk = __builtin_ctz(i + 1), k = b + 1 + kk;
+        const std::vector<Stmt> st = stmts_for(P.touched[k]);
+        const size_t first = items.size();
+        step_base = "jt" + std::to_string(next_step_id);
+        step_items(items, step_base, kk + 1 < u ? off_const(k, ((i + 1) >> (kk + 1)) & 1u) : off_dyn(k, "ngh"),
+                   P.touched[k], false, b, kHiStep, &st);
+        own_base(first);
+        items.push_back({accumulate_text(false, 0u), {}});
+        items.push_back({"tot += acc;", {}});
+        items.push_back({"acc = 0.0;", {}});
+        body[kCenAcc] += 1.0, body[kCenLane] += 1.0;
+      }
+      emit_items(items, ind);
+      o << ind << "}\n";
+    }
+    body[kCenAcc] += 1.0;
+    if (Q > U) {
+      std::vector<int> rows;
+      {
+        std::vector<char> in(P.n, 0);
+        for (int k = b + u + 1; k < m; ++k)
+          for (int r : P.touched[k]) in[r] = 1;
+        for (int r = 0; r < P.n; ++r)
+          if (in[r]) rows.push_back(r);
+      }
+      const std::vector<Stmt> st = stmts_for(rows);
+      o << ind << "if (qq + 1u < " << Q / U << "u) {\n";
+      o << ind << "  const char* jt = (const char*)opaque_c(p.jtab, 0u);\n";
+      o << ind << "  const uint32_t kk = (uint32_t)__builtin_ctz(qq + 1u);\n";
+      o << ind << "  const uint32_t ngd = ((qq + 1u) >> (kk + 1u)) & 1u;\n";
+      std::vector<Item> items;
+      step_items(items, "(const char*)opaque_c(p.cols, 0u)",
+                 "(2u * (" + std::to_string(L + b + 1 + u) + "u + kk) + ngd) * " + std::to_string(P.NP * 8) + "u",
+                 rows, true, b, kSharedStep, &st);
+      items.push_back({accumulate_text(false, 0u), {}});
+      emit_items(items, "          ");
+      o << ind << "  tot += acc;\n" << ind << "  acc = 0.0;\n";
+      body[kCenLane] += 1.0;
+      o << ind << "}\n";
+    }
+    o << "      }\n";
   }
 
   std::string source() {
@@ -1211,6 +1338,7 @@
     o << "      const uint64_t a = base + j;\n";
     o << "      if (a >= p.chunk_count) break;\n";
     o << "      const uint64_t ga = p.chunk_begin + a;\n";
+    const size_t start_begin = o.str().size();
     o << "      double x[N], y[" << len0 << "];\n";
     if (trace) o << "      const uint64_t tr_s = __builtin_amdgcn_s_memtime();\n";
     o << "      chunk_start" << (P.start_tab_on ? "_tab" : "") << "<N>(x, p, ga, SUP_LANE());\n";
@@ -1258,6 +1386,12 @@
     }
     o << "      double tot = 0.0;\n";
     if (trace) o << "      asm volatile(\"\" : \"+v\"(acc));\n      tr_sc += __builtin_amdgcn_s_memtime() - tr_s;\n      ++tr_n;\n";
+    const int u = std::max(0, std::min(P.seg_hi, m - 1 - b));
+    const unsigned U = 1u << u;
+    const size_t start_end = o.str().size();
+    if (u > 0) {
+      hi_loop(Q, U, u);
+    } else {
     o << "      for (uint32_t q = 0; q < " << Q << "u; ++q) {\n";
     const char* ind = "        ";
     o << ind << "const char* jt = (const char*)opaque_c(p.jtab, 0u);\n";
@@ -1270,9 +1404,11 @@
           step_items(items, "jt", pb < b - 1 ? off_const(k, (st >> (pb + 1)) & 1u) : off_dyn(k, "ng"),
                      P.touched[k], false, step_class(k, b));
         items.push_back({accumulate_text(st & 1u, state(st)), {}});
+        body[kCenAcc] += 1.0;
       }
       emit_items(items, ind);
     }
+    body[kCenAcc] += 1.0;
     if (Q > 1) {
       o << ind << "if (q + 1u < " << Q << "u) {\n";
       o << ind << "  const uint32_t kk = (uint32_t)__builtin_ctz(q + 1u);\n";
@@ -1281,14 +1417,27 @@
         std::vector<Item> items;
         step_items(items, "(const char*)opaque_c(p.cols, 0u)",
                    "(2u * (" + std::to_string(L + b + 1) + "u + kk) + ngd) * " + std::to_string(P.NP * 8) + "u",
-                   P.dyn_rows, true, P.seg_b);
+                   P.dyn_rows, true, P.seg_b, kSharedStep);
         items.push_back({accumulate_text(false, 0u), {}});
         emit_items(items, "          ");
       }
       o << ind << "  tot += acc;\n" << ind << "  acc = 0.0;\n";
+      body[kCenLane] += 1.0;
       o << ind << "}\n";
     }
     o << "      }\n";
+    }
+    {
+      const double steps = 2.0 * (double)U * (double)B;
+      double walk = 0.0;
+      for (int c = 0; c < kCenStart; ++c) census[c] = body[c] / steps, walk += body[c];
+      const std::string init = o.str().substr(start_begin, start_end - start_begin);
+      const double start_ops = count_sub(init, " + ") + count_sub(init, " * ") + count_sub(init, " - ") +
+                               count_sub(init, "__builtin_fma(") + 7.0 +
+                               (double)n * ((double)L + (P.start_tab_on ? 0.0 : 0.5 * (double)(n - 1 - L - m)));
+      census[kCenStart] = std::ldexp(start_ops, -m);
+      block_bytes = 1.25 * 8.0 * walk;
+    }
     o << "      acc = tot + acc;\n";
     o << "      if (((uint32_t)ga ^ (uint32_t)__builtin_popcount(SUP_LANE())) & 1u) acc = -acc;\n";
     o << "      }\n";
@@ -1401,7 +1550,7 @@
   });
 }
 
-int build_seg(Plan& P, int fixed_budget) {
+int build_seg(Plan& P, int fixed_budget, int fixed_hi) {
   const int n = P.n, L = P.lay.L, m = P.lay.m;
   if (m < 3) {
     set_error("segmented walk needs >= 3 walk bits");
@@ -1478,7 +1627,7 @@
   SR.len0 = P.seg_start[1], SR.s_end = P.sub_start.back(), SR.r_end = P.seg_start.back();
   seg_rows_finish(SR, P.seg_b);
   const int cc_cap = std::min(max_cached(), P.lay.cc_cap);
-  auto finish = [&SR, &cc_cap, n, L, m](Plan& Q, int budget) {
+  auto finish = [&SR, &cc_cap, n, L, m](Plan& Q, int budget, int hi) {
     SegFit f;
     if (const char* e = std::getenv("SUP_JIT_CC"))
       f = seg_fit(SR, std::max(0, std::min({std::atoi(e), SR.b - 1, kMaxCachedBits})), budget);
@@ -1487,7 +1636,7 @@
     Q.outer_tree = std::move(f.outer);
     Q.inner_tree = std::move(f.inner);
     Q.seg_cc = f.cc;
-    Q.seg_ops = f.ops;
+    Q.seg_model_ops = f.ops;
     Q.seg_regs = f.regs;
     Q.seg_budget = budget;
     Q.jofs.assign(m, 0);
@@ -1505,18 +1654,47 @@
     Q.seg_cbase = Q.jtab.size();
     Q.seg_kp = 4;
     if (const char* e = std::getenv("SUP_JIT_KP")) Q.seg_kp = std::max(1, std::atoi(e));
-    Gen g(Q);
-    Q.jit_src = g.source();
+    const int hi_max = std::min(3, m - 1 - Q.seg_b);
+    if (const char* e = std::getenv("SUP_JIT_HI")) hi = std::max(0, std::min(3, std::atoi(e)));
+    bool neg_zero = false;
+    for (int j = 0; j < n; ++j) neg_zero = neg_zero || (Q.x0[j] == 0.0 && std::signbit(Q.x0[j]));
+    if (neg_zero) hi = 0;
+    auto generate = [&Q](int h, std::string* src) {
+      Q.seg_hi = h;
+      auto g = std::make_unique<Gen>(Q);
+      *src = g->source();
+      return g;
+    };
+    auto total = [](const Gen& g) {
+      double ops = 0.0;
+      for (int c = 0; c < kCenStart; ++c) ops += g.census[c];
+      return ops;
+    };
+    int taken = hi < 0 ? 0 : std::min(hi, hi_max);
+    std::string src;
+    std::unique_ptr<Gen> g = generate(taken, &src);
+    for (int h = hi < 0 ? hi_max : 0; h > 0; --h) {
+      std::string s2;
+      std::unique_ptr<Gen> gh = generate(h, &s2);
+      if (gh->block_bytes <= kMaxBlockBytes && total(*gh) < total(*g)) {
+        g = std::move(gh), src = std::move(s2), taken = h;
+        break;
+      }
+    }
+    Q.seg_hi = taken;
+    Q.jit_src = std::move(src);
+    for (int c = 0; c < kSegCensusN; ++c) Q.seg_census[c] = g->census[c];
+    Q.seg_ops = total(*g);
     {
-      const std::vector<double> t = g.tail();
+      const std::vector<double> t = g->tail();
       Q.jtab.insert(Q.jtab.end(), t.begin(), t.end());
     }
     Q.jit_key = jit_source_key(Q.jit_src);
-    (void)n;
   };
   const char* env_budget = std::getenv("SUP_JIT_BUDGET");
+  const int hi_unchecked = fixed_budget > 0 ? fixed_hi : 0;
   if (env_budget) fixed_budget = std::max(1, std::atoi(env_budget));
-  finish(P, fixed_budget > 0 ? fixed_budget : kRegsMax);
+  finish(P, fixed_budget > 0 ? fixed_budget : kRegsMax, hi_unchecked);
   const bool fixed = fixed_budget > 0 || std::getenv("SUP_JIT_REGMAX") || std::getenv("SUP_JIT_STORAGE") ||
                      std::getenv("SUP_JIT_CC") || std::getenv("SUP_JIT_NOVERIFY");
   const double walk_s = std::ldexp(1.0, n - 1) * P.seg_ops / 3.7e13;
@@ -1530,11 +1708,11 @@
     CodeScan s;
     P.seg_loop_scratch = jit_code_scan(P, &s) != SUP_OK || s.loop_scratch != 0;
   }
-  if (!fixed && walk_s >= 0.01 && P.seg_regs > kRegs3) {
+  auto ladder = [&](int hi, Plan& out) -> int {
     std::vector<int> budgets;
     for (int b2 = kRegs3 + 20; b2 <= kRegsMax + 60; b2 += 8) budgets.push_back(b2);
     std::vector<Plan> cand(budgets.size(), P);
-    parallel_tasks(budgets.size(), [&](size_t i) { finish(cand[i], budgets[i]); });
+    parallel_tasks(budgets.size(), [&](size_t i) { finish(cand[i], budgets[i], hi); });
     std::vector<size_t> idx;
     for (size_t i = 0; i < cand.size(); ++i) {
       bool dup = false;
@@ -1622,7 +1800,7 @@
                    : scans[k].scratch_bytes ? kCleanScratch
                                             : kClean0;
     }
-    if (outcome[idx[pp]] == kFail) return SUP_EHIP;
+    if (outcome[idx[pp]] == kFail) return (int)SUP_EHIP;
     auto pick = [&]() {
       int c = -1, bare = -1;
       for (size_t i : idx) {
@@ -1636,15 +1814,37 @@
     if (std::getenv("SUP_JIT_VERBOSE"))
       for (size_t i : idx)
         if (done[i])
-          std::fprintf(stderr, "  budget %d: ops %.4f rc %d vgprs %d spills %d scratch %dB (loop %d of %d insts, %d readlane)%s\n",
-                       budgets[i], cand[i].seg_ops, src[i], scans[i].vgprs, scans[i].vgpr_spills,
+          std::fprintf(stderr, "  budget %d hi %d: ops %.4f rc %d vgprs %d spills %d scratch %dB (loop %d of %d insts, %d readlane)%s\n",
+                       budgets[i], cand[i].seg_hi, cand[i].seg_ops, src[i], scans[i].vgprs, scans[i].vgpr_spills,
                        scans[i].scratch_bytes, scans[i].loop_scratch, scans[i].loop_insts, scans[i].loop_readlane,
                        (int)i == best ? "  <- chosen" : "");
     if (best < 0) {
       set_error("segmented walk: every budget's kernel touches scratch inside its walk loop (or fails to compile)");
-      return SUP_EHIP;
-    }
-    P = std::move(cand[best]);
+      return (int)SUP_EHIP;
+    }
+    out = std::move(cand[best]);
+    return SUP_OK;
+  };
+  if (!fixed && walk_s >= 0.01 && P.seg_regs > kRegs3) {
+    Plan best_hi, best_0;
+    const int rc_hi = ladder(-1, best_hi);
+    int rc_0 = SUP_EHIP;
+    bool need_0 = rc_hi != SUP_OK || best_hi.seg_hi == 0;
+    if (!need_0) {
+      Plan top = P;
+      finish(top, kRegsMax + 60, 0);
+      need_0 = top.seg_ops <= best_hi.seg_ops;
+    }
+    if (rc_hi == SUP_OK && best_hi.seg_hi == 0) rc_0 = SUP_OK, best_0 = best_hi, need_0 = false;
+    else if (need_0) rc_0 = ladder(0, best_0);
+    if (rc_hi != SUP_OK && rc_0 != SUP_OK) return SUP_EHIP;
+    const bool take_hi = rc_hi == SUP_OK && (rc_0 != SUP_OK || best_hi.seg_ops < best_0.seg_ops);
+    if (std::getenv("SUP_JIT_VERBOSE"))
+      std::fprintf(stderr, "  high-bit steps: %s (unrolled ladder %s hi %d ops %.4f; plain ladder %s ops %.4f)\n",
+                   take_hi ? "taken" : "not taken", rc_hi == SUP_OK ? "ok" : "failed", best_hi.seg_hi,
+                   rc_hi == SUP_OK ? best_hi.seg_ops : 0.0,
+                   rc_0 == SUP_OK ? "ok" : (need_0 ? "failed" : "not needed"), rc_0 == SUP_OK ? best_0.seg_ops : 0.0);
+    P = std::move(take_hi ? best_hi : best_0);
   }
   P.seg_skip = seg_skip_fraction_plan(P, 2048);
   if (P.start_tab_on) seg_start_table(P);
@@ -1653,6 +1853,17 @@
                  "(storage plans evaluated: %ld)\n", n, m, P.seg_b, P.seg_ops, P.seg_regs, P.seg_cc,
                  P.jtab.size() * sizeof(double), P.seg_cbase * sizeof(double), (unsigned long long)P.jit_key,
                  g_fit_calls.load());
+  if (std::getenv("SUP_JIT_VERBOSE")) {
+    const double* c = P.seg_census;
+    std::fprintf(stderr,
+                 "  op census (fp64 ops per Gray step, hi=%d): x adds %.4f, copy adds %.4f, outer forms %.4f, "
+                 "segment-0 forms %.4f, D %.4f, accumulates %.4f, lane sum %.4f, shared step adds %.4f copies %.4f "
+                 "forms %.4f, high-bit steps adds %.4f copies %.4f forms %.4f; total %.4f (storage fit's count of the "
+                 "plain walk loop without the lane sum %.4f); beside it, chunk start %.4f\n",
+                 P.seg_hi, c[kCenXAdd], c[kCenCopy], c[kCenOuter], c[kCenInner], c[kCenD], c[kCenAcc], c[kCenLane],
+                 c[kCenSharedAdd], c[kCenSharedCopy], c[kCenSharedForm], c[kCenHiAdd], c[kCenHiCopy], c[kCenHiForm],
+                 P.seg_ops, P.seg_model_ops, c[kCenStart]);
+  }
   return SUP_OK;
 }
 
diff --git a/superman_amd/csrc/jit_compile.cpp b/superman_amd/csrc/jit_compile.cpp
--- a/superman_amd/csrc/jit_compile.cpp
+++ b/superman_amd/csrc/jit_compile.cpp
@@ -420,8 +420,8 @@
   std::istringstream in(buf.data());
   std::string tag;
   int ver = 0, cnt = 0;
-  if (!(in >> tag >> ver >> *m >> c->b >> c->budget >> c->cc_cap >> cnt) || tag != "supseg" || ver != 3 || cnt < 1 ||
-      cnt > 64 || c->cc_cap < 0 || c->cc_cap > kMaxCachedBits)
+  if (!(in >> tag >> ver >> *m >> c->b >> c->budget >> c->cc_cap >> c->hi >> cnt) || tag != "supseg" || ver != 4 || cnt < 1 ||
+      cnt > 64 || c->hi < 0 || c->hi > 3 || c->cc_cap < 0 || c->cc_cap > kMaxCachedBits)
     return false;
   c->order.resize(cnt);
   for (int& v : c->order)
@@ -439,7 +439,7 @@
   const std::string dir = cache_dir();
   if (dir.empty() || c.order.empty()) return;
   std::ostringstream o;
-  o << "supseg 3 " << m << ' ' << c.b << ' ' << c.budget << ' ' << c.cc_cap << ' ' << c.order.size();
+  o << "supseg 4 " << m << ' ' << c.b << ' ' << c.budget << ' ' << c.cc_cap << ' ' << c.hi << ' ' << c.order.size();
   for (int v : c.order) o << ' ' << v;
   o << '\n';
   const std::string str = o.str();
diff --git a/superman_amd/csrc/plan.cpp b/superman_amd/csrc/plan.cpp
--- a/superman_amd/csrc/plan.cpp
+++ b/superman_amd/csrc/plan.cpp
@@ -463,7 +463,7 @@
     if ((kind == kWalkSparse || kind == kWalkDense) && !lane_touched && rm == 0 && !no_chunk_ends())
       P.chunk_ends |= 1ull << j;
   }
-  if (kind == kWalkSeg) return build_seg(P, choice ? choice->budget : 0);
+  if (kind == kWalkSeg) return build_seg(P, choice ? choice->budget : 0, choice ? choice->hi : 0);
   return SUP_OK;
 }
 
@@ -541,7 +541,7 @@
   if (!lay.fixed) {
     const int mmax = std::min(lay.m + lay.h - kSegMinChunkBits, 31);
     int m2 = lay.m;
-    while (m2 < mmax && std::ldexp(walk_cost(P), m2) < 32.0 * kSegStartOps) ++m2;
+    while (m2 < mmax && std::ldexp(P.seg_model_ops, m2) < 32.0 * kSegStartOps) ++m2;
     if (m2 != lay.m) {
       Layout l2 = lay;
       l2.m = m2;
@@ -549,7 +549,7 @@
       Plan s2;
       if (plan(l2, s2) == SUP_OK) {
         auto eff = [](const Plan& q) {
-          return (1.0 - q.seg_skip) * (walk_cost(q) + std::ldexp(kSegStartOps, -q.lay.m));
+          return (1.0 - q.seg_skip) * (q.seg_model_ops + std::ldexp(kSegStartOps, -q.lay.m));
         };
         if (eff(s2) < eff(P)) P = std::move(s2);
       }
@@ -559,6 +559,7 @@
   c.order = P.seg_order;
   c.b = P.seg_b;
   c.budget = P.seg_budget;
+  c.hi = P.seg_hi;
   c.cc_cap = P.lay.cc_cap;
   seg_choice_store(dkey, P.lay.m, c);
   const double cold_s = std::chrono::duration<double>(std::chrono::steady_clock::now() - t_cold).count();
```

After: 3241 billion gray-steps/s (median of 6 runs). 1.03x the previous value.
